# chaitjo/efficient-gnns

Hardware: NVIDIA H100
Metric: edges aggregated/s (fwd+bwd), 3-layer GCN student + logit-KD, ARXIV-shape (higher is better)
Workload: dtype f32

## Files before the change

### efficient-gnns_b200/csrc/common.cuh

```cuda
#pragma once
#include <cuda_runtime.h>
#include <stdint.h>

#include "b200gnn.h"

namespace b200gnn {

void set_cuda_error(cudaError_t e);
void count_launch(int n = 1);

inline int check_launch() {
  cudaError_t e = cudaGetLastError();
  if (e != cudaSuccess) {
    set_cuda_error(e);
    return B200GNN_ERR_CUDA;
  }
  count_launch();
  return B200GNN_OK;
}

constexpr unsigned FULL_MASK = 0xffffffffu;

__device__ __forceinline__ void adam_update(float& p, float& m, float& v, float g, float b1, float b2, float eps,
                                            float step_size, float inv_sqrt_bc2) {
  const float mi = b1 * m + (1.f - b1) * g;
  const float vi = b2 * v + (1.f - b2) * g * g;
  m = mi; v = vi;
  p -= step_size * mi / (sqrtf(vi) * inv_sqrt_bc2 + eps);
}

template <typename V> struct VecTraits;
template <> struct VecTraits<float> { static constexpr int W = 1; };
template <> struct VecTraits<float2> { static constexpr int W = 2; };
template <> struct VecTraits<float4> { static constexpr int W = 4; };

__device__ __forceinline__ void vzero(float& a) { a = 0.f; }
__device__ __forceinline__ void vzero(float2& a) { a.x = a.y = 0.f; }
__device__ __forceinline__ void vzero(float4& a) { a.x = a.y = a.z = a.w = 0.f; }

__device__ __forceinline__ void vfma(float& acc, float s, const float& x) { acc = fmaf(s, x, acc); }
__device__ __forceinline__ void vfma(float2& acc, float s, const float2& x) {
  acc.x = fmaf(s, x.x, acc.x); acc.y = fmaf(s, x.y, acc.y);
}
__device__ __forceinline__ void vfma(float4& acc, float s, const float4& x) {
  acc.x = fmaf(s, x.x, acc.x); acc.y = fmaf(s, x.y, acc.y);
  acc.z = fmaf(s, x.z, acc.z); acc.w = fmaf(s, x.w, acc.w);
}
__device__ __forceinline__ void vadd(float& a, const float& b) { a += b; }
__device__ __forceinline__ void vadd(float2& a, const float2& b) { a.x += b.x; a.y += b.y; }
__device__ __forceinline__ void vadd(float4& a, const float4& b) {
  a.x += b.x; a.y += b.y; a.z += b.z; a.w += b.w;
}
__device__ __forceinline__ void vdiv(float& a, float d) { a /= d; }
__device__ __forceinline__ void vdiv(float2& a, float d) { a.x /= d; a.y /= d; }
__device__ __forceinline__ void vdiv(float4& a, float d) { a.x /= d; a.y /= d; a.z /= d; a.w /= d; }
__device__ __forceinline__ void vstat(float& s, float& q, const float& y) { s += y; q = fmaf(y, y, q); }
__device__ __forceinline__ void vstat(float2& s, float2& q, const float2& y) {
  s.x += y.x; s.y += y.y; q.x = fmaf(y.x, y.x, q.x); q.y = fmaf(y.y, y.y, q.y);
}
__device__ __forceinline__ void vstat(float4& s, float4& q, const float4& y) {
  s.x += y.x; s.y += y.y; s.z += y.z; s.w += y.w;
  q.x = fmaf(y.x, y.x, q.x); q.y = fmaf(y.y, y.y, q.y);
  q.z = fmaf(y.z, y.z, q.z); q.w = fmaf(y.w, y.w, q.w);
}

__device__ __forceinline__ float vshfl_down(float v, int d) { return __shfl_down_sync(FULL_MASK, v, d); }
__device__ __forceinline__ float2 vshfl_down(float2 v, int d) {
  return make_float2(__shfl_down_sync(FULL_MASK, v.x, d), __shfl_down_sync(FULL_MASK, v.y, d));
}
__device__ __forceinline__ float4 vshfl_down(float4 v, int d) {
  return make_float4(__shfl_down_sync(FULL_MASK, v.x, d), __shfl_down_sync(FULL_MASK, v.y, d),
                     __shfl_down_sync(FULL_MASK, v.z, d), __shfl_down_sync(FULL_MASK, v.w, d));
}

__device__ __forceinline__ float vldg(const float* p) { return __ldg(p); }
__device__ __forceinline__ float2 vldg(const float2* p) { return __ldg(p); }
__device__ __forceinline__ float4 vldg(const float4* p) { return __ldg(p); }

__device__ __forceinline__ void vstcs(float* p, const float& v) { __stcs(p, v); }
__device__ __forceinline__ void vstcs(float2* p, const float2& v) { __stcs(p, v); }
__device__ __forceinline__ void vstcs(float4* p, const float4& v) { __stcs(p, v); }

static __global__ void __launch_bounds__(256) sum_partials_kernel(const float* __restrict__ partial, int n, double scale,
                                                                  float* __restrict__ out) {
  __shared__ double s[256];
  double a = 0.0;
  for (int i = threadIdx.x; i < n; i += 256) a += (double)partial[i];
  s[threadIdx.x] = a;
  __syncthreads();
  for (int d = 128; d > 0; d >>= 1) {
    if (threadIdx.x < d) s[threadIdx.x] += s[threadIdx.x + d];
    __syncthreads();
  }
  if (threadIdx.x == 0) out[0] = (float)(s[0] * scale);
}

inline bool aligned_to(const void* p, size_t a) { return (reinterpret_cast<uintptr_t>(p) % a) == 0; }

}
```

### efficient-gnns_b200/csrc/dense_rows.cu

```cuda
#include "common.cuh"
#include "philox.cuh"

namespace b200gnn {

constexpr int ROWS_THREADS = 256;

struct RowMap {
  int nvec, rows_per_iter, cv, rg;
  bool active;
};
__device__ __forceinline__ RowMap make_row_map(int K) {
  RowMap m;
  m.nvec = K >> 2;
  m.rows_per_iter = ROWS_THREADS / m.nvec;
  m.rg = threadIdx.x / m.nvec;
  m.cv = threadIdx.x - m.rg * m.nvec;
  m.active = m.rg < m.rows_per_iter;
  return m;
}

__device__ __forceinline__ float4 ld4(const float* p) { return *reinterpret_cast<const float4*>(p); }
__device__ __forceinline__ float4 ld4s(const float* p) { return __ldcs(reinterpret_cast<const float4*>(p)); }
__device__ __forceinline__ void st4(float* p, const float4& v) { *reinterpret_cast<float4*>(p) = v; }

__device__ __forceinline__ void reduce_store_2xK(const RowMap& m, int K, float4 a, float4 b, float* smem ,
                                                 float* out) {
  for (int i = threadIdx.x; i < 2 * K; i += ROWS_THREADS) smem[i] = 0.f;
  __syncthreads();
  for (int g = 0; g < m.rows_per_iter; ++g) {
    if (m.active && m.rg == g) {
      float* s = smem + 4 * m.cv;
      float* q = smem + K + 4 * m.cv;
      s[0] += a.x; s[1] += a.y; s[2] += a.z; s[3] += a.w;
      q[0] += b.x; q[1] += b.y; q[2] += b.z; q[3] += b.w;
    }
    __syncthreads();
  }
  for (int i = threadIdx.x; i < 2 * K; i += ROWS_THREADS) out[i] = smem[i];
}

__global__ void __launch_bounds__(ROWS_THREADS) col_stats4_kernel(const float* __restrict__ Y, int64_t n_rows, int K,
                                                                  float* __restrict__ partial, int slots) {
  extern __shared__ float smem[];
  const RowMap m = make_row_map(K);
  const int64_t per = (n_rows + slots - 1) / slots;
  const int64_t r0 = (int64_t)blockIdx.x * per, r1 = min(n_rows, r0 + per);
  float4 s = make_float4(0, 0, 0, 0), q = s;
  if (m.active)
    for (int64_t r = r0 + m.rg; r < r1; r += m.rows_per_iter) {
      const float4 y = ld4(Y + (size_t)r * K + 4 * m.cv);
      vstat(s, q, y);
    }
  reduce_store_2xK(m, K, s, q, smem, partial + (size_t)blockIdx.x * 2 * K);
}

constexpr int FIN_COLS = 4, FIN_GROUPS = 64;
__device__ __forceinline__ bool finalize_reduce(const float* __restrict__ partial, int slots, int K, bool second,
                                                double& s_out, double& q_out, int& k_out) {
  __shared__ double sh[2][FIN_GROUPS][FIN_COLS];
  const int c = threadIdx.x % FIN_COLS, g = threadIdx.x / FIN_COLS;
  const int k = blockIdx.x * FIN_COLS + c;
  double s = 0.0, q = 0.0;
  if (k < K)
    for (int j = g; j < slots; j += FIN_GROUPS) {
      s += (double)partial[(size_t)j * 2 * K + k];
      if (second) q += (double)partial[(size_t)j * 2 * K + K + k];
    }
  sh[0][g][c] = s; sh[1][g][c] = q;
  __syncthreads();
  if (g == 0 && k < K) {
    s = 0.0; q = 0.0;
    for (int j = 0; j < FIN_GROUPS; ++j) { s += sh[0][j][c]; q += sh[1][j][c]; }
    s_out = s; q_out = q; k_out = k;
    return true;
  }
  return false;
}

__global__ void __launch_bounds__(256) bn_finalize_kernel(const float* __restrict__ partial, int slots, int K,
                                                          int64_t n, const float* __restrict__ gamma,
                                                          const float* __restrict__ beta, float eps, float momentum,
                                                          float* running_mean, float* running_var, float* mean_out,
                                                          float* invstd_out, float* scale_out, float* shift_out) {
  double s, q; int k;
  if (finalize_reduce(partial, slots, K, true, s, q, k)) {
    const double mean = s / (double)n;
    double var = q / (double)n - mean * mean;
    if (var < 0.0) var = 0.0;
    const float invstd = (float)(1.0 / sqrt(var + (double)eps));
    const float sc = gamma[k] * invstd;
    mean_out[k] = (float)mean;
    invstd_out[k] = invstd;
    scale_out[k] = sc;
    shift_out[k] = beta[k] - (float)mean * sc;
    if (running_mean) {
      const double unbiased = n > 1 ? var * (double)n / (double)(n - 1) : var;
      running_mean[k] = (1.f - momentum) * running_mean[k] + momentum * (float)mean;
      running_var[k] = (1.f - momentum) * running_var[k] + momentum * (float)unbiased;
    }
  }
}

__device__ __forceinline__ float4 affine_relu4(float4 y, const float* __restrict__ scale, const float* __restrict__ shift,
                                               int cv, int relu) {
  if (scale) {
    const float4 sc = ld4(scale + 4 * cv), sh = ld4(shift + 4 * cv);
    y.x = fmaf(y.x, sc.x, sh.x); y.y = fmaf(y.y, sc.y, sh.y);
    y.z = fmaf(y.z, sc.z, sh.z); y.w = fmaf(y.w, sc.w, sh.w);
  }
  if (relu) { y.x = fmaxf(y.x, 0.f); y.y = fmaxf(y.y, 0.f); y.z = fmaxf(y.z, 0.f); y.w = fmaxf(y.w, 0.f); }
  return y;
}

template <bool P16>
__global__ void __launch_bounds__(256) affine_relu_dropout_kernel(const float* __restrict__ Y, float* __restrict__ out,
                                                                  int64_t n_vec, int nvec_row,
                                                                  const float* __restrict__ scale,
                                                                  const float* __restrict__ shift, int relu, float p,
                                                                  uint32_t thr16, uint64_t seed, uint64_t offset,
                                                                  const int32_t* __restrict__ step_dev,
                                                                  uint64_t step_mul, uint64_t index_offset) {
  const float inv_keep = p > 0.f ? 1.f / (1.f - p) : 1.f;
  if (step_dev) offset += (uint64_t)(*step_dev) * step_mul;
  const int64_t tid = (int64_t)blockIdx.x * blockDim.x + threadIdx.x, stride = (int64_t)gridDim.x * blockDim.x;
  if (P16) {
    const uint64_t g0 = index_offset, g1 = index_offset + (uint64_t)n_vec;
    for (uint64_t b = (g0 >> 1) + (uint64_t)tid; b < ((g1 + 1) >> 1); b += (uint64_t)stride) {
      const uint4 r = philox4x32(seed, offset, b);
#pragma unroll
      for (int half = 0; half < 2; ++half) {
        const uint64_t g = 2 * b + half;
        if (g < g0 || g >= g1) continue;
        const int64_t i = (int64_t)(g - g0);
        float4 y = affine_relu4(ld4s(Y + 4 * i), scale, shift, (int)(i % nvec_row), relu);
        const uchar4 m = keep16(half ? r.z : r.x, half ? r.w : r.y, thr16);
        y.x = m.x ? y.x * inv_keep : 0.f; y.y = m.y ? y.y * inv_keep : 0.f;
        y.z = m.z ? y.z * inv_keep : 0.f; y.w = m.w ? y.w * inv_keep : 0.f;
        st4(out + 4 * i, y);
      }
    }
  } else {
    for (int64_t i = tid; i < n_vec; i += stride) {
      float4 y = affine_relu4(ld4s(Y + 4 * i), scale, shift, (int)(i % nvec_row), relu);
      if (p > 0.f) {
        const uchar4 m = keep24(philox4x32(seed, offset, (uint64_t)i + index_offset), p);
        y.x = m.x ? y.x * inv_keep : 0.f; y.y = m.y ? y.y * inv_keep : 0.f;
        y.z = m.z ? y.z * inv_keep : 0.f; y.w = m.w ? y.w * inv_keep : 0.f;
      }
      st4(out + 4 * i, y);
    }
  }
}

struct RowScatter {
  float* ptr[16];
  int32_t off[17];
  int32_t n;
  int64_t ld, col;
};
__device__ __forceinline__ float* scatter_row(const RowScatter& sc, int64_t r) {
  int q = 0;
#pragma unroll 1
  while (q + 1 < sc.n && r >= sc.off[q + 1]) ++q;
  return sc.ptr[q] + (size_t)(r - sc.off[q]) * (size_t)sc.ld + sc.col;
}

template <bool P16>
__global__ void __launch_bounds__(256) affine_relu_dropout_mapped_kernel(
    const float* __restrict__ Y, float* __restrict__ out, int64_t n_rows, int nvec_l, const float* __restrict__ scale,
    const float* __restrict__ shift, int relu, float p, uint32_t thr16, uint64_t seed, uint64_t offset,
    const int32_t* __restrict__ step_dev, uint64_t step_mul, const int32_t* __restrict__ rowmap, uint64_t row_offset,
    uint64_t nvec_g, uint64_t cv_off, int paired, const RowScatter sc) {
  const float inv_keep = p > 0.f ? 1.f / (1.f - p) : 1.f;
  if (step_dev) offset += (uint64_t)(*step_dev) * step_mul;
  const int64_t tid = (int64_t)blockIdx.x * blockDim.x + threadIdx.x, stride = (int64_t)gridDim.x * blockDim.x;
  if (P16 && paired) {
    const int half_l = nvec_l >> 1;
    for (int64_t u = tid; u < n_rows * half_l; u += stride) {
      const int64_t r = u / half_l;
      const int cv = (int)(u - r * half_l) * 2;
      const uint64_t gid = rowmap ? (uint64_t)rowmap[r] : (uint64_t)r + row_offset;
      const uint64_t g = gid * nvec_g + cv_off + (uint64_t)cv;
      const uint4 rnd = philox4x32(seed, offset, g >> 1);
#pragma unroll
      for (int half = 0; half < 2; ++half) {
        const int64_t i = r * nvec_l + cv + half;
        float4 y = affine_relu4(ld4s(Y + 4 * i), scale, shift, cv + half, relu);
        const uchar4 m = keep16(half ? rnd.z : rnd.x, half ? rnd.w : rnd.y, thr16);
        y.x = m.x ? y.x * inv_keep : 0.f; y.y = m.y ? y.y * inv_keep : 0.f;
        y.z = m.z ? y.z * inv_keep : 0.f; y.w = m.w ? y.w * inv_keep : 0.f;
        st4(out + 4 * i, y);
        if (sc.n) st4(scatter_row(sc, r) + 4 * (cv + half), y);
      }
    }
    return;
  }
  for (int64_t i = tid; i < n_rows * nvec_l; i += stride) {
    const int64_t r = i / nvec_l;
    const int cv = (int)(i - r * nvec_l);
    float4 y = affine_relu4(ld4s(Y + 4 * i), scale, shift, cv, relu);
    if (p > 0.f) {
      const uint64_t gid = rowmap ? (uint64_t)rowmap[r] : (uint64_t)r + row_offset;
      const uint64_t g = gid * nvec_g + cv_off + (uint64_t)cv;
      uchar4 m;
      if (P16) {
        const uint4 rnd = philox4x32(seed, offset, g >> 1);
        m = keep16((g & 1) ? rnd.z : rnd.x, (g & 1) ? rnd.w : rnd.y, thr16);
      } else {
        m = keep24(philox4x32(seed, offset, g), p);
      }
      y.x = m.x ? y.x * inv_keep : 0.f; y.y = m.y ? y.y * inv_keep : 0.f;
      y.z = m.z ? y.z * inv_keep : 0.f; y.w = m.w ? y.w * inv_keep : 0.f;
    }
    st4(out + 4 * i, y);
    if (sc.n) st4(scatter_row(sc, r) + 4 * cv, y);
  }
}

__global__ void __launch_bounds__(256) dropout_mask_kernel(uint8_t* __restrict__ mask, int64_t n_vec, float p, int p16,
                                                           uint32_t thr16, uint64_t seed, uint64_t offset) {
  for (int64_t i = (int64_t)blockIdx.x * blockDim.x + threadIdx.x; i < n_vec; i += (int64_t)gridDim.x * blockDim.x) {
    uchar4 m;
    if (p16) {
      const uint4 r = philox4x32(seed, offset, (uint64_t)i >> 1);
      m = keep16((i & 1) ? r.z : r.x, (i & 1) ? r.w : r.y, thr16);
    } else {
      m = keep24(philox4x32(seed, offset, (uint64_t)i), p);
    }
    reinterpret_cast<uchar4*>(mask)[i] = m;
  }
}

__global__ void __launch_bounds__(256) dropout_bits_kernel(uint32_t* __restrict__ bits, int n_layers, int64_t n_rows, int nvec_row,
                                                           int words, float p, int p16, uint32_t thr16, uint64_t seed,
                                                           uint64_t offset, const int32_t* __restrict__ step_dev,
                                                           uint64_t step_mul) {
  if (step_dev) offset += (uint64_t)(*step_dev) * step_mul;
  const int64_t per_layer = n_rows * words;
  for (int64_t t = (int64_t)blockIdx.x * blockDim.x + threadIdx.x; t < per_layer * n_layers; t += (int64_t)gridDim.x * blockDim.x) {
    const int layer = (int)(t / per_layer);
    const int64_t e = t - layer * per_layer, row = e / words;
    const int w = (int)(e - row * words);
    const uint64_t off = offset + (uint64_t)layer;
    uint32_t out = 0u;
    uint64_t blk = ~0ull;
    uint4 r = make_uint4(0u, 0u, 0u, 0u);
#pragma unroll
    for (int j = 0; j < 8; ++j) {
      const int cv = 8 * w + j;
      if (cv >= nvec_row) break;
      const uint64_t g = (uint64_t)row * nvec_row + cv;
      uchar4 m;
      if (p16) {
        if ((g >> 1) != blk) { blk = g >> 1; r = philox4x32(seed, off, blk); }
        m = keep16((g & 1) ? r.z : r.x, (g & 1) ? r.w : r.y, thr16);
      } else {
        m = keep24(philox4x32(seed, off, g), p);
      }
      out |= ((uint32_t)m.x | ((uint32_t)m.y << 1) | ((uint32_t)m.z << 2) | ((uint32_t)m.w << 3)) << (4 * j);
    }
    bits[t] = out;
  }
}

__global__ void __launch_bounds__(256) affine_relu_bits_kernel(const float* __restrict__ Y, const uint32_t* __restrict__ bits,
                                                               const float* __restrict__ scale, const float* __restrict__ shift,
                                                               float* __restrict__ out, int64_t n_vec, int nvec_row, int words,
                                                               float p) {
  const float inv_keep = p > 0.f ? 1.f / (1.f - p) : 1.f;
  for (int64_t i = (int64_t)blockIdx.x * blockDim.x + threadIdx.x; i < n_vec; i += (int64_t)gridDim.x * blockDim.x) {
    const int64_t row = i / nvec_row;
    const int cv = (int)(i - row * nvec_row);
    float4 y = affine_relu4(ld4(Y + 4 * i), scale, shift, cv, 1);
    const uint32_t b = bits[row * words + (cv >> 3)] >> (4 * (cv & 7));
    y.x = (b & 1u) ? y.x * inv_keep : 0.f; y.y = (b & 2u) ? y.y * inv_keep : 0.f;
    y.z = (b & 4u) ? y.z * inv_keep : 0.f; y.w = (b & 8u) ? y.w * inv_keep : 0.f;
    st4(out + 4 * i, y);
  }
}

__global__ void __launch_bounds__(256) relu_dropout_bwd_kernel(const float4* __restrict__ dOut, const float4* __restrict__ Xout,
                                                               float4* dY, int64_t n_vec, float inv_keep) {
  for (int64_t i = (int64_t)blockIdx.x * blockDim.x + threadIdx.x; i < n_vec; i += (int64_t)gridDim.x * blockDim.x) {
    const float4 g = dOut[i], x = Xout[i];
    float4 d;
    d.x = x.x > 0.f ? g.x * inv_keep : 0.f; d.y = x.y > 0.f ? g.y * inv_keep : 0.f;
    d.z = x.z > 0.f ? g.z * inv_keep : 0.f; d.w = x.w > 0.f ? g.w * inv_keep : 0.f;
    dY[i] = d;
  }
}

__global__ void __launch_bounds__(ROWS_THREADS) bn_act_bwd_reduce_kernel(
    const float* __restrict__ dOut, const float* __restrict__ Xout, const float* __restrict__ Y,
    const float* __restrict__ mean, const float* __restrict__ invstd, int64_t n_rows, int K, float inv_keep,
    float* __restrict__ partial, int slots) {
  extern __shared__ float smem[];
  const RowMap m = make_row_map(K);
  const int64_t per = (n_rows + slots - 1) / slots;
  const int64_t r0 = (int64_t)blockIdx.x * per, r1 = min(n_rows, r0 + per);
  float4 s = make_float4(0, 0, 0, 0), q = s;
  if (m.active) {
    const float4 mu = ld4(mean + 4 * m.cv), is = ld4(invstd + 4 * m.cv);
    for (int64_t r = r0 + m.rg; r < r1; r += m.rows_per_iter) {
      const size_t o = (size_t)r * K + 4 * m.cv;
      const float4 g = ld4(dOut + o), x = ld4(Xout + o), y = ld4(Y + o);
      const float dx = x.x > 0.f ? g.x * inv_keep : 0.f, dy = x.y > 0.f ? g.y * inv_keep : 0.f;
      const float dz = x.z > 0.f ? g.z * inv_keep : 0.f, dw = x.w > 0.f ? g.w * inv_keep : 0.f;
      s.x += dx; s.y += dy; s.z += dz; s.w += dw;
      q.x = fmaf(dx, (y.x - mu.x) * is.x, q.x); q.y = fmaf(dy, (y.y - mu.y) * is.y, q.y);
      q.z = fmaf(dz, (y.z - mu.z) * is.z, q.z); q.w = fmaf(dw, (y.w - mu.w) * is.w, q.w);
    }
  }
  reduce_store_2xK(m, K, s, q, smem, partial + (size_t)blockIdx.x * 2 * K);
}

__global__ void __launch_bounds__(256) bn_bwd_finalize_kernel(const float* __restrict__ partial, int slots, int K,
                                                              int64_t n, const float* __restrict__ gamma,
                                                              const float* __restrict__ invstd, float* dgamma,
                                                              float* dbeta, float* coef ) {
  double s, q; int k;
  if (finalize_reduce(partial, slots, K, true, s, q, k)) {
    dbeta[k] = (float)s;
    dgamma[k] = (float)q;
    coef[k] = gamma[k] * invstd[k];
    coef[K + k] = (float)(s / (double)n);
    coef[2 * K + k] = (float)(q / (double)n);
  }
}

template <bool DZ>
__global__ void __launch_bounds__(ROWS_THREADS) bn_act_bwd_apply_kernel(
    const float* __restrict__ dOut, const float* __restrict__ Xout, const float* __restrict__ Y,
    const float* __restrict__ mean, const float* __restrict__ invstd, const float* __restrict__ coef, int64_t n_rows,
    int K, float inv_keep, float* __restrict__ dY, float* __restrict__ colsum_partial, int slots) {
  extern __shared__ float smem[];
  const RowMap m = make_row_map(K);
  const int64_t per = (n_rows + slots - 1) / slots;
  const int64_t r0 = (int64_t)blockIdx.x * per, r1 = min(n_rows, r0 + per);
  float4 s = make_float4(0, 0, 0, 0), q = s;
  if (m.active) {
    const float4 mu = ld4(mean + 4 * m.cv), is = ld4(invstd + 4 * m.cv);
    const float4 c1 = ld4(coef + 4 * m.cv), c2 = ld4(coef + K + 4 * m.cv), c3 = ld4(coef + 2 * K + 4 * m.cv);
    for (int64_t r = r0 + m.rg; r < r1; r += m.rows_per_iter) {
      const size_t o = (size_t)r * K + 4 * m.cv;
      float4 g = ld4s(dOut + o);
      const float4 y = ld4s(Y + o);
      if (!DZ) {
        const float4 x = ld4s(Xout + o);
        g.x = x.x > 0.f ? g.x * inv_keep : 0.f; g.y = x.y > 0.f ? g.y * inv_keep : 0.f;
        g.z = x.z > 0.f ? g.z * inv_keep : 0.f; g.w = x.w > 0.f ? g.w * inv_keep : 0.f;
      }
      float4 d;
      d.x = c1.x * (g.x - c2.x - (y.x - mu.x) * is.x * c3.x);
      d.y = c1.y * (g.y - c2.y - (y.y - mu.y) * is.y * c3.y);
      d.z = c1.z * (g.z - c2.z - (y.z - mu.z) * is.z * c3.z);
      d.w = c1.w * (g.w - c2.w - (y.w - mu.w) * is.w * c3.w);
      st4(dY + o, d);
      s.x += d.x; s.y += d.y; s.z += d.z; s.w += d.w;
    }
  }
  if (colsum_partial) reduce_store_2xK(m, K, s, q, smem, colsum_partial + (size_t)blockIdx.x * 2 * K);
}

__global__ void __launch_bounds__(256) partial_reduce_kernel(const float* __restrict__ partial, int slots, int K2,
                                                             float* __restrict__ out) {
  __shared__ double sh[FIN_GROUPS][FIN_COLS];
  const int c = threadIdx.x % FIN_COLS, g = threadIdx.x / FIN_COLS;
  const int k = blockIdx.x * FIN_COLS + c;
  double s = 0.0;
  if (k < K2)
    for (int j = g; j < slots; j += FIN_GROUPS) s += (double)partial[(size_t)j * K2 + k];
  sh[g][c] = s;
  __syncthreads();
  if (g == 0 && k < K2) {
    s = 0.0;
    for (int j = 0; j < FIN_GROUPS; ++j) s += sh[j][c];
    out[k] = (float)s;
  }
}

__global__ void __launch_bounds__(256) colsum_finalize_kernel(const float* __restrict__ partial, int slots, int K,
                                                              float* __restrict__ out) {
  double s, q; int k;
  if (finalize_reduce(partial, slots, K, false, s, q, k)) out[k] = (float)s;
}

__global__ void __launch_bounds__(256) adam_kernel(float* __restrict__ p, const float* __restrict__ g,
                                                   float* __restrict__ m, float* __restrict__ v, int64_t n, float lr,
                                                   float b1, float b2, float eps, const int32_t* __restrict__ step) {
  const float t = (float)(*step + 1);
  const float bc1 = 1.f - powf(b1, t), bc2 = 1.f - powf(b2, t);
  const float step_size = lr / bc1, inv_sqrt_bc2 = rsqrtf(bc2);
  for (int64_t i = (int64_t)blockIdx.x * blockDim.x + threadIdx.x; i < n; i += (int64_t)gridDim.x * blockDim.x)
    adam_update(p[i], m[i], v[i], g[i], b1, b2, eps, step_size, inv_sqrt_bc2);
}
__global__ void adam_tick_kernel(int32_t* step) { *step += 1; }

static inline int grid_for(int64_t n_items, int per_cta, int cap = 132 * 8) {
  int64_t g = (n_items + per_cta - 1) / per_cta;
  if (g > cap) g = cap;
  if (g < 1) g = 1;
  return (int)g;
}

}

using namespace b200gnn;

static bool rows_ok(int64_t n_rows, int64_t K) { return n_rows >= 0 && K > 0 && K % 4 == 0 && K <= 1024; }

extern "C" int64_t b200gnn_rows_slots(int64_t n_rows) {
  int64_t s = (n_rows + 255) / 256;
  if (s > 132 * 4) s = 132 * 4;
  return s < 1 ? 1 : s;
}

extern "C" int b200gnn_col_stats_f32(const float* Y, int64_t n_rows, int64_t K, float* partial, int64_t slots,
                                     void* stream) {
  if (!rows_ok(n_rows, K) || !Y || !partial || slots < 1 || !aligned_to(Y, 16)) return B200GNN_ERR_BAD_ARG;
  col_stats4_kernel<<<(int)slots, ROWS_THREADS, 2 * K * sizeof(float), (cudaStream_t)stream>>>(Y, n_rows, (int)K, partial,
                                                                                             (int)slots);
  return check_launch();
}

extern "C" int b200gnn_bn_finalize_f32(const float* partial, int64_t slots, int64_t K, int64_t n_rows,
                                       const float* gamma, const float* beta, float eps, float momentum,
                                       float* running_mean, float* running_var, float* mean_out, float* invstd_out,
                                       float* scale_out, float* shift_out, void* stream) {
  if (!partial || slots < 1 || K <= 0 || n_rows <= 0 || !gamma || !beta || !mean_out || !invstd_out || !scale_out ||
      !shift_out || ((running_mean == nullptr) != (running_var == nullptr)))
    return B200GNN_ERR_BAD_ARG;
  bn_finalize_kernel<<<(int)((K + FIN_COLS - 1) / FIN_COLS), 256, 0, (cudaStream_t)stream>>>(
      partial, (int)slots, (int)K, n_rows, gamma, beta, eps, momentum, running_mean, running_var, mean_out, invstd_out,
      scale_out, shift_out);
  return check_launch();
}

extern "C" int b200gnn_affine_relu_dropout_f32(const float* Y, float* out, int64_t n_rows, int64_t K,
                                               const float* scale, const float* shift, int relu, float p, uint64_t seed,
                                               uint64_t offset, const int32_t* step_dev, uint64_t step_mul,
                                               uint64_t row_offset, void* stream) {
  if (!rows_ok(n_rows, K) || !Y || !out || p < 0.f || p >= 1.f || ((scale == nullptr) != (shift == nullptr)) ||
      !aligned_to(Y, 16) || !aligned_to(out, 16))
    return B200GNN_ERR_BAD_ARG;
  if (n_rows == 0) return B200GNN_OK;
  const int64_t n_vec = n_rows * (K / 4);
  uint32_t thr16 = 0;
  if (dropout_p16(p, thr16))
    affine_relu_dropout_kernel<true><<<grid_for((n_vec + 1) / 2 + 1, 256 * 2), 256, 0, (cudaStream_t)stream>>>(
        Y, out, n_vec, (int)(K / 4), scale, shift, relu, p, thr16, seed, offset, step_dev, step_mul,
        row_offset * (uint64_t)(K / 4));
  else
    affine_relu_dropout_kernel<false><<<grid_for(n_vec, 256 * 4), 256, 0, (cudaStream_t)stream>>>(
        Y, out, n_vec, (int)(K / 4), scale, shift, relu, p, 0u, seed, offset, step_dev, step_mul,
        row_offset * (uint64_t)(K / 4));
  return check_launch();
}

static int mapped_launch(const float* Y, float* out, int64_t n_rows, int64_t K, const float* scale, const float* shift, int relu,
                         float p, uint64_t seed, uint64_t offset, const int32_t* step_dev, uint64_t step_mul, const int32_t* rowmap,
                         uint64_t row_offset, int64_t K_global, int64_t col_offset, const RowScatter& sc, void* stream) {
  if (!rows_ok(n_rows, K) || !Y || !out || p < 0.f || p >= 1.f || ((scale == nullptr) != (shift == nullptr)) ||
      !aligned_to(Y, 16) || !aligned_to(out, 16) || K_global < K || K_global % 4 || col_offset < 0 || col_offset % 4 ||
      col_offset + K > K_global)
    return B200GNN_ERR_BAD_ARG;
  if (n_rows == 0) return B200GNN_OK;
  const int nvec_l = (int)(K / 4);
  const uint64_t nvec_g = (uint64_t)(K_global / 4), cv_off = (uint64_t)(col_offset / 4);
  const int paired = (nvec_l % 2 == 0 && nvec_g % 2 == 0 && cv_off % 2 == 0) ? 1 : 0;
  const int64_t n_vec = n_rows * nvec_l;
  uint32_t thr16 = 0;
  if (dropout_p16(p, thr16))
    affine_relu_dropout_mapped_kernel<true><<<grid_for(paired ? n_vec / 2 : n_vec, 256 * 2), 256, 0, (cudaStream_t)stream>>>(
        Y, out, n_rows, nvec_l, scale, shift, relu, p, thr16, seed, offset, step_dev, step_mul, rowmap, row_offset, nvec_g,
        cv_off, paired, sc);
  else
    affine_relu_dropout_mapped_kernel<false><<<grid_for(n_vec, 256 * 4), 256, 0, (cudaStream_t)stream>>>(
        Y, out, n_rows, nvec_l, scale, shift, relu, p, 0u, seed, offset, step_dev, step_mul, rowmap, row_offset, nvec_g,
        cv_off, 0, sc);
  return check_launch();
}

extern "C" int b200gnn_affine_relu_dropout_mapped_f32(const float* Y, float* out, int64_t n_rows, int64_t K,
                                                      const float* scale, const float* shift, int relu, float p,
                                                      uint64_t seed, uint64_t offset, const int32_t* step_dev,
                                                      uint64_t step_mul, const int32_t* rowmap, uint64_t row_offset,
                                                      int64_t K_global, int64_t col_offset, void* stream) {
  RowScatter sc;
  sc.n = 0; sc.ld = 0; sc.col = 0;
  return mapped_launch(Y, out, n_rows, K, scale, shift, relu, p, seed, offset, step_dev, step_mul, rowmap, row_offset, K_global,
                       col_offset, sc, stream);
}

extern "C" int b200gnn_affine_relu_dropout_scatter_f32(const float* Y, float* out, int64_t n_rows, int64_t K,
                                                       const float* scale, const float* shift, int relu, float p,
                                                       uint64_t seed, uint64_t offset, const int32_t* step_dev,
                                                       uint64_t step_mul, const int32_t* rowmap, uint64_t row_offset,
                                                       int64_t K_global, int64_t col_offset, float* const* dst_ptrs,
                                                       const int32_t* row_off, int32_t world, int64_t ld_dst, void* stream) {
  if (!dst_ptrs || !row_off || world <= 0 || world > 16 || ld_dst < K_global || ld_dst % 4 || row_off[0] != 0 ||
      row_off[world] != n_rows)
    return B200GNN_ERR_BAD_ARG;
  RowScatter sc;
  sc.n = world; sc.ld = ld_dst; sc.col = col_offset;
  for (int q = 0; q < world; ++q) {
    if (!dst_ptrs[q] || !aligned_to(dst_ptrs[q], 16) || row_off[q + 1] < row_off[q]) return B200GNN_ERR_BAD_ARG;
    sc.ptr[q] = dst_ptrs[q]; sc.off[q] = row_off[q];
  }
  sc.off[world] = row_off[world];
  return mapped_launch(Y, out, n_rows, K, scale, shift, relu, p, seed, offset, step_dev, step_mul, rowmap, row_offset, K_global,
                       col_offset, sc, stream);
}

extern "C" int b200gnn_dropout_mask_u8(uint8_t* mask, int64_t n_rows, int64_t K, float p, uint64_t seed,
                                       uint64_t offset, void* stream) {
  if (!rows_ok(n_rows, K) || !mask || p < 0.f || p >= 1.f) return B200GNN_ERR_BAD_ARG;
  if (n_rows == 0) return B200GNN_OK;
  const int64_t n_vec = n_rows * (K / 4);
  uint32_t thr16 = 0;
  const int p16 = dropout_p16(p, thr16) ? 1 : 0;
  dropout_mask_kernel<<<grid_for(n_vec, 256 * 4), 256, 0, (cudaStream_t)stream>>>(mask, n_vec, p, p16, thr16, seed, offset);
  return check_launch();
}

extern "C" int b200gnn_dropout_bits_u32(uint32_t* bits, int64_t n_layers, int64_t n_rows, int64_t K, float p, uint64_t seed,
                                        uint64_t offset, const int32_t* step_dev, uint64_t step_mul, void* stream) {
  if (!rows_ok(n_rows, K) || !bits || n_layers < 1 || p < 0.f || p >= 1.f) return B200GNN_ERR_BAD_ARG;
  if (n_rows == 0) return B200GNN_OK;
  const int words = (int)((K + 31) / 32);
  uint32_t thr16 = 0;
  const int p16 = dropout_p16(p, thr16) ? 1 : 0;
  dropout_bits_kernel<<<grid_for(n_layers * n_rows * words, 256 * 2), 256, 0, (cudaStream_t)stream>>>(
      bits, (int)n_layers, n_rows, (int)(K / 4), words, p, p16, thr16, seed, offset, step_dev, step_mul);
  return check_launch();
}

extern "C" int b200gnn_affine_relu_bits_f32(const float* Y, const uint32_t* bits, const float* scale, const float* shift,
                                            float p, float* out, int64_t n_rows, int64_t K, void* stream) {
  if (!rows_ok(n_rows, K) || !Y || !bits || !scale || !shift || !out || p < 0.f || p >= 1.f || !aligned_to(Y, 16) ||
      !aligned_to(out, 16) || !aligned_to(scale, 16) || !aligned_to(shift, 16))
    return B200GNN_ERR_BAD_ARG;
  if (n_rows == 0) return B200GNN_OK;
  const int64_t n_vec = n_rows * (K / 4);
  affine_relu_bits_kernel<<<grid_for(n_vec, 256 * 4), 256, 0, (cudaStream_t)stream>>>(Y, bits, scale, shift, out, n_vec,
                                                                                     (int)(K / 4), (int)((K + 31) / 32), p);
  return check_launch();
}

extern "C" int b200gnn_relu_dropout_bwd_f32(const float* dOut, const float* Xout, float* dY, int64_t n_rows, int64_t K,
                                            float p, void* stream) {
  if (!rows_ok(n_rows, K) || p < 0.f || p >= 1.f) return B200GNN_ERR_BAD_ARG;
  if (n_rows == 0) return B200GNN_OK;
  if (!dOut || !Xout || !dY || !aligned_to(dOut, 16) || !aligned_to(Xout, 16) || !aligned_to(dY, 16)) return B200GNN_ERR_BAD_ARG;
  const int64_t n_vec = n_rows * (K / 4);
  const float inv_keep = p > 0.f ? 1.f / (1.f - p) : 1.f;
  relu_dropout_bwd_kernel<<<grid_for(n_vec, 256 * 4), 256, 0, (cudaStream_t)stream>>>(
      reinterpret_cast<const float4*>(dOut), reinterpret_cast<const float4*>(Xout), reinterpret_cast<float4*>(dY), n_vec, inv_keep);
  return check_launch();
}

extern "C" int b200gnn_bn_act_bwd_reduce_f32(const float* dOut, const float* Xout, const float* Y, const float* mean,
                                             const float* invstd, int64_t n_rows, int64_t K, float p, float* partial,
                                             int64_t slots, void* stream) {
  if (!rows_ok(n_rows, K) || n_rows == 0 || !dOut || !Xout || !Y || !mean || !invstd || !partial || slots < 1 ||
      p < 0.f || p >= 1.f)
    return B200GNN_ERR_BAD_ARG;
  if (ROWS_THREADS / (K / 4) < 1) return B200GNN_ERR_UNSUPPORTED;
  const float inv_keep = p > 0.f ? 1.f / (1.f - p) : 1.f;
  bn_act_bwd_reduce_kernel<<<(int)slots, ROWS_THREADS, 2 * K * sizeof(float), (cudaStream_t)stream>>>(
      dOut, Xout, Y, mean, invstd, n_rows, (int)K, inv_keep, partial, (int)slots);
  return check_launch();
}

extern "C" int b200gnn_bn_act_bwd_apply_f32(const float* dOut, const float* Xout, const float* Y, const float* mean,
                                            const float* invstd, const float* gamma, const float* sums,
                                            int64_t sum_slots, int64_t n_norm, int64_t n_rows, int64_t K, float p,
                                            float* dY, float* dgamma, float* dbeta, float* dbias, float* partial,
                                            int64_t slots, float* coef, void* stream) {
  if (!rows_ok(n_rows, K) || n_rows == 0 || !dOut || !Y || !mean || !invstd || !gamma || !sums || !dY ||
      !dgamma || !dbeta || !partial || !coef || slots < 1 || sum_slots < 1 || n_norm < 1 || p < 0.f || p >= 1.f)
    return B200GNN_ERR_BAD_ARG;
  cudaStream_t st = (cudaStream_t)stream;
  const float inv_keep = p > 0.f ? 1.f / (1.f - p) : 1.f;
  const size_t smem = 2 * K * sizeof(float);
  int rc;
  bn_bwd_finalize_kernel<<<(int)((K + FIN_COLS - 1) / FIN_COLS), 256, 0, st>>>(sums, (int)sum_slots, (int)K, n_norm, gamma,
                                                                              invstd, dgamma, dbeta, coef);
  if ((rc = check_launch())) return rc;
  if (Xout)
    bn_act_bwd_apply_kernel<false><<<(int)slots, ROWS_THREADS, smem, st>>>(dOut, Xout, Y, mean, invstd, coef, n_rows, (int)K,
                                                                          inv_keep, dY, dbias ? partial : nullptr, (int)slots);
  else
    bn_act_bwd_apply_kernel<true><<<(int)slots, ROWS_THREADS, smem, st>>>(dOut, nullptr, Y, mean, invstd, coef, n_rows, (int)K,
                                                                         inv_keep, dY, dbias ? partial : nullptr, (int)slots);
  if ((rc = check_launch())) return rc;
  if (dbias) {
    colsum_finalize_kernel<<<(int)((K + FIN_COLS - 1) / FIN_COLS), 256, 0, st>>>(partial, (int)slots, (int)K, dbias);
    if ((rc = check_launch())) return rc;
  }
  return B200GNN_OK;
}

extern "C" int b200gnn_bn_act_bwd_f32(const float* dOut, const float* Xout, const float* Y, const float* mean,
                                      const float* invstd, const float* gamma, int64_t n_rows, int64_t K, float p,
                                      float* dY, float* dgamma, float* dbeta, float* dbias, float* partial,
                                      int64_t slots, float* coef, void* stream) {
  int rc = b200gnn_bn_act_bwd_reduce_f32(dOut, Xout, Y, mean, invstd, n_rows, K, p, partial, slots, stream);
  if (rc) return rc;
  return b200gnn_bn_act_bwd_apply_f32(dOut, Xout, Y, mean, invstd, gamma, partial, slots, n_rows, n_rows, K, p, dY,
                                      dgamma, dbeta, dbias, partial, slots, coef, stream);
}

extern "C" int b200gnn_partial_reduce_f32(const float* partial, int64_t slots, int64_t K2, float* out, void* stream) {
  if (!partial || !out || slots < 1 || K2 < 1) return B200GNN_ERR_BAD_ARG;
  partial_reduce_kernel<<<(int)((K2 + FIN_COLS - 1) / FIN_COLS), 256, 0, (cudaStream_t)stream>>>(partial, (int)slots, (int)K2,
                                                                                               out);
  return check_launch();
}

extern "C" int b200gnn_col_sum_f32(const float* Y, int64_t n_rows, int64_t K, float* out, float* partial,
                                   int64_t slots, void* stream) {
  if (!rows_ok(n_rows, K) || !Y || !out || !partial || slots < 1) return B200GNN_ERR_BAD_ARG;
  cudaStream_t st = (cudaStream_t)stream;
  int rc;
  col_stats4_kernel<<<(int)slots, ROWS_THREADS, 2 * K * sizeof(float), st>>>(Y, n_rows, (int)K, partial, (int)slots);
  if ((rc = check_launch())) return rc;
  colsum_finalize_kernel<<<(int)((K + FIN_COLS - 1) / FIN_COLS), 256, 0, st>>>(partial, (int)slots, (int)K, out);
  return check_launch();
}

extern "C" int b200gnn_adam_step_f32(float* params, const float* grads, float* exp_avg, float* exp_avg_sq, int64_t n,
                                     float lr, float beta1, float beta2, float eps, int32_t* step, void* stream) {
  if (!params || !grads || !exp_avg || !exp_avg_sq || !step || n < 0) return B200GNN_ERR_BAD_ARG;
  cudaStream_t st = (cudaStream_t)stream;
  int rc;
  if (n > 0) {
    adam_kernel<<<grid_for(n, 256), 256, 0, st>>>(params, grads, exp_avg, exp_avg_sq, n, lr, beta1, beta2, eps, step);
    if ((rc = check_launch())) return rc;
  }
  adam_tick_kernel<<<1, 1, 0, st>>>(step);
  return check_launch();
}
```

### efficient-gnns_b200/csrc/gemm_wgrad_tf32x3.cu

```cuda
#include "common.cuh"
#include "tc_common.cuh"

namespace b200gnn {
namespace wgrad {
using namespace tc;

constexpr int BKN = 32;
constexpr int TM = 128, TN = 128;
constexpr int THREADS = 384;
constexpr int STAGES = 5;
constexpr int X_BOX = 8;
constexpr int RAW_BYTES = BKN * (TM + TN) * 4;
constexpr int OP_BYTES = 128 * BKN * 4;
constexpr int T_BYTES = 2 * OP_BYTES;
constexpr int SS_BYTES = TM / 2 * 16;
constexpr int SMEM_BYTES = STAGES * RAW_BYTES + 2 * T_BYTES + 256 + SS_BYTES + 1024;
constexpr int MAX_RANGES = 132;
constexpr int64_t MAX_PARTIAL_FLOATS = (int64_t)MAX_RANGES * 256 * 256;
constexpr int MAX_KIN = 2048, MAX_NOUT = 512;
static_assert(SMEM_BYTES <= 232448, "shared memory");

struct Params {
  float* partial;
  int32_t Nn, Kin, Kpad, Nout, Npad, num_kb;
  int32_t n_tn, n_ranges;
  const float* act_scale;
  const float* act_shift;
  const uint32_t* act_bits;
  int32_t act_words;
  float inv_keep;
  const float* act_slope;
  int32_t act_ld;
};

template <bool ACT, bool PRELU = false>
__global__ void __launch_bounds__(THREADS, 1)
wgrad_tf32x3_kernel(const __grid_constant__ CUtensorMap tmX, const __grid_constant__ CUtensorMap tmG, const Params p) {
  extern __shared__ uint8_t smem_raw[];
  uint8_t* smem = reinterpret_cast<uint8_t*>((reinterpret_cast<uintptr_t>(smem_raw) + 1023) & ~(uintptr_t)1023);
  uint8_t* tbuf = smem + STAGES * RAW_BYTES;
  uint64_t* full = reinterpret_cast<uint64_t*>(tbuf + 2 * T_BYTES);
  uint64_t* empty = full + STAGES;
  float4* act_ss = reinterpret_cast<float4*>(tbuf + 2 * T_BYTES + 256);

  const int tiles = (p.Kpad / TM) * p.n_tn;
  const int tile = (int)blockIdx.x % tiles, range = (int)blockIdx.x / tiles;
  const int mt = tile / p.n_tn, nt = tile % p.n_tn;
  const int kb0 = (int)((int64_t)p.num_kb * range / p.n_ranges);
  const int kb1 = (int)((int64_t)p.num_kb * (range + 1) / p.n_ranges);

  const int warp = threadIdx.x >> 5, lane = threadIdx.x & 31;
  if (threadIdx.x == 0) {
    for (int s = 0; s < STAGES; ++s) { mbar_init(&full[s], 1); mbar_init(&empty[s], 256); }
    asm volatile("fence.mbarrier_init.release.cluster;" ::: "memory");
  }
  __syncthreads();

  if (warp < 4) {
    regs_dec<40>();
    if (threadIdx.x == 0) {
      int s = 0; uint32_t ph = 0;
      for (int kb = kb0; kb < kb1; ++kb) {
        mbar_wait(&empty[s], ph ^ 1);
        uint8_t* st = smem + s * RAW_BYTES;
        mbar_expect_tx(&full[s], RAW_BYTES);
        for (int j = 0; j < TM / X_BOX; ++j)
          tma_load_2d(&tmX, &full[s], st + j * BKN * X_BOX * 4, mt * TM + j * X_BOX, kb * BKN);
        tma_load_2d(&tmG, &full[s], st + BKN * TM * 4, nt * TN, kb * BKN);
        if (++s == STAGES) { s = 0; ph ^= 1; }
      }
    }
    return;
  }
  regs_inc<232>();

  const int cw = (warp >> 2) - 1;
  const int ct = threadIdx.x - 128;
  const uint32_t xfrag = (8 * cw + 2 * (warp & 3)) * (BKN * X_BOX * 4) + (lane & 3) * (X_BOX * 4) + (lane >> 2) * 4;
  const int pair = cw * 32 + (warp & 3) * 8 + (lane >> 2);
  const int c0 = mt * TM + cw * 64 + (warp & 3) * 16 + (lane >> 2);
  uint32_t wnext = 0u;
  const int bits_ld = PRELU ? p.act_ld : p.act_words;
  auto act_word = [&](int kb) {
    const int node = kb * BKN + lane;
    return node < p.Nn && (c0 >> 5) < p.act_words ? __ldg(p.act_bits + (size_t)node * bits_ld + (c0 >> 5)) : 0u;
  };
  const float slope = PRELU ? __ldg(p.act_slope) : 0.f;
  if (PRELU && kb0 < kb1) wnext = act_word(kb0);
  if (ACT) {
    if (ct < TM / 2) {
      const int c = mt * TM + (ct >> 3) * 16 + (ct & 7);
      float4 v = make_float4(0.f, 0.f, 0.f, 0.f);
      if (c < p.Kin) { v.x = __ldg(p.act_scale + c); v.y = __ldg(p.act_shift + c); }
      if (c + 8 < p.Kin) { v.z = __ldg(p.act_scale + c + 8); v.w = __ldg(p.act_shift + c + 8); }
      act_ss[ct] = v;
    }
    if (kb0 < kb1) wnext = act_word(kb0);
    named_sync(1, 256);
  }
  float acc[64], sum[64];
#pragma unroll
  for (int i = 0; i < 64; ++i) sum[i] = acc[i] = 0.f;
  uint32_t xh0[BKN / 8][4], xl0[BKN / 8][4], xh1[BKN / 8][4], xl1[BKN / 8][4];
  int s = 0; uint32_t ph = 0;
  auto block = [&](int i, uint32_t (&h)[BKN / 8][4], uint32_t (&l)[BKN / 8][4]) {
    uint32_t wcur = 0u;
    if (ACT || PRELU) {
      wcur = wnext;
      if (kb0 + i + 1 < kb1) wnext = act_word(kb0 + i + 1);
    }
    mbar_wait(&full[s], ph);
    float4 ss = make_float4(0.f, 0.f, 0.f, 0.f);
    int l4 = lane & 3;
    if (ACT) {
      ss = act_ss[pair];
      asm volatile("" : "+r"(l4));
    }
    if (PRELU) asm volatile("" : "+r"(l4));
    const uint32_t sraw = smem_u32(smem + s * RAW_BYTES);
    const float* rg = reinterpret_cast<const float*>(smem + s * RAW_BYTES + BKN * TM * 4);
    uint8_t* T = tbuf + (i & 1) * T_BYTES;
#pragma unroll
    for (int u = 0; u < 4; ++u) {
      const int idx = u * 256 + ct;
      const int r = idx & 127, c = idx >> 7;
      const float* src = rg + (4 * c) * 128 + r;
      const uint4 v = make_uint4(__float_as_uint(src[0]), __float_as_uint(src[128]), __float_as_uint(src[256]),
                                 __float_as_uint(src[384]));
      uint4 hv, lv;
      split4(v, hv, lv);
      *reinterpret_cast<uint4*>(T + swz128(r, c)) = hv;
      *reinterpret_cast<uint4*>(T + OP_BYTES + swz128(r, c)) = lv;
    }
#pragma unroll
    for (int k = 0; k < BKN / 8; ++k)
#pragma unroll
      for (int j = 0; j < 4; ++j) {
        uint32_t v = lds32(sraw + xfrag + (j & 1) * (BKN * X_BOX * 4) + (8 * k + 4 * (j >> 1)) * (X_BOX * 4));
        if (ACT) {
          const uint32_t w = __shfl_sync(0xffffffffu, wcur, 8 * k + l4 + 4 * (j >> 1));
          const float y = fmaxf(fmaf(__uint_as_float(v), (j & 1) ? ss.z : ss.x, (j & 1) ? ss.w : ss.y), 0.f) * p.inv_keep;
          v = (w >> ((c0 & 31) + 8 * (j & 1))) & 1u ? __float_as_uint(y) : 0u;
        }
        if (PRELU) {
          const uint32_t w = __shfl_sync(0xffffffffu, wcur, 8 * k + l4 + 4 * (j >> 1));
          const float z = __uint_as_float(v);
          const float y = (z > 0.f ? z : slope * z) * p.inv_keep;
          v = (w >> ((c0 & 31) + 8 * (j & 1))) & 1u ? __float_as_uint(y) : 0u;
        }
        split1(v, h[k][j], l[k][j]);
      }
    asm volatile("fence.proxy.async.shared::cta;" ::: "memory");
    mbar_arrive(&empty[s]);
    if (i > 0) {
      wgmma_wait<0>();
      acc_fence(acc);
#pragma unroll
      for (int j = 0; j < 64; ++j) sum[j] += acc[j];
    }
    named_sync(1, 256);
    reg_fence(h); reg_fence(l);
    wgmma_fence();
    const uint32_t sa = smem_u32(T);
#pragma unroll
    for (int k = 0; k < BKN / 8; ++k) {
      const uint32_t koff = k * 32;
      wgmma_tf32_n128_rs(acc, l[k], make_desc_k128(sa + koff), k != 0);
      wgmma_tf32_n128_rs(acc, h[k], make_desc_k128(sa + OP_BYTES + koff), 1);
    }
#pragma unroll
    for (int k = 0; k < BKN / 8; ++k) wgmma_tf32_n128_rs(acc, h[k], make_desc_k128(sa + k * 32), 1);
    wgmma_commit();
    if (++s == STAGES) { s = 0; ph ^= 1; }
  };
  for (int i = 0; i < kb1 - kb0; i += 2) {
    block(i, xh0, xl0);
    if (i + 1 < kb1 - kb0) block(i + 1, xh1, xl1);
  }
  if (kb1 > kb0) {
    wgmma_wait<0>();
    acc_fence(acc);
#pragma unroll
    for (int j = 0; j < 64; ++j) sum[j] += acc[j];
  }
  float* out = p.partial + (size_t)range * p.Kpad * p.Npad;
  const int row0 = mt * TM + cw * 64 + (warp & 3) * 16 + (lane >> 2);
#pragma unroll
  for (int j = 0; j < 16; ++j) {
    const int col = nt * TN + 8 * j + 2 * (lane & 3);
    if (col < p.Npad) {
      *reinterpret_cast<float2*>(out + (size_t)row0 * p.Npad + col) = make_float2(sum[4 * j], sum[4 * j + 1]);
      *reinterpret_cast<float2*>(out + (size_t)(row0 + 8) * p.Npad + col) = make_float2(sum[4 * j + 2], sum[4 * j + 3]);
    }
  }
}

constexpr int RED_VECS = 32, RED_GROUPS = 8;
__global__ void __launch_bounds__(RED_VECS * RED_GROUPS) wgrad_reduce_kernel(const float4* __restrict__ partial, int n_part,
                                                                             int Kin, int Kpad, int Nout, int Npad,
                                                                             float* __restrict__ out) {
  __shared__ float4 sh[RED_GROUPS][RED_VECS];
  const int64_t n_vec = (int64_t)Kpad * Npad / 4;
  const int v = threadIdx.x % RED_VECS, g = threadIdx.x / RED_VECS;
  const int64_t i = (int64_t)blockIdx.x * RED_VECS + v;
  float4 acc = make_float4(0.f, 0.f, 0.f, 0.f);
  if (i < n_vec)
    for (int c = g; c < n_part; c += RED_GROUPS) {
      const float4 x = __ldcs(partial + (size_t)c * n_vec + i);
      acc.x += x.x; acc.y += x.y; acc.z += x.z; acc.w += x.w;
    }
  sh[g][v] = acc;
  __syncthreads();
  if (g != 0 || i >= n_vec) return;
  const int row = (int)(i / (Npad / 4)), c4 = (int)(i % (Npad / 4)) * 4;
  if (c4 >= Nout || row >= Kin) return;
#pragma unroll
  for (int j = 1; j < RED_GROUPS; ++j) {
    const float4 x = sh[j][v];
    acc.x += x.x; acc.y += x.y; acc.z += x.z; acc.w += x.w;
  }
  *reinterpret_cast<float4*>(out + (size_t)row * Nout + c4) = acc;
}

static bool make_map_rows(CUtensorMap* m, const float* base, int64_t rows, int64_t width, int64_t ld, int box_cols) {
  EncodeTiledFn fn = encode_fn();
  if (!fn) return false;
  cuuint64_t dims[2] = {(cuuint64_t)width, (cuuint64_t)rows};
  cuuint64_t strides[1] = {(cuuint64_t)ld * 4};
  cuuint32_t box[2] = {(cuuint32_t)box_cols, (cuuint32_t)BKN};
  cuuint32_t estr[2] = {1, 1};
  return fn(m, CU_TENSOR_MAP_DATA_TYPE_FLOAT32, 2, const_cast<float*>(base), dims, strides, box, estr,
            CU_TENSOR_MAP_INTERLEAVE_NONE, CU_TENSOR_MAP_SWIZZLE_NONE, CU_TENSOR_MAP_L2_PROMOTION_L2_256B,
            CU_TENSOR_MAP_FLOAT_OOB_FILL_NONE) == CUDA_SUCCESS;
}

static int64_t pad_k(int64_t Kin) { return (Kin + TM - 1) / TM * TM; }
static int64_t pad_n(int64_t Nout) { return (Nout + 31) / 32 * 32; }
static int range_cap(int64_t Kin, int64_t Nout) {
  const int64_t c = MAX_PARTIAL_FLOATS / (pad_k(Kin) * pad_n(Nout));
  return (int)(c > MAX_RANGES ? MAX_RANGES : (c < 1 ? 1 : c));
}

}
}

using namespace b200gnn;

extern "C" int64_t b200gnn_wgrad_workspace_floats(int64_t Kin, int64_t Nout) {
  if (Kin <= 0 || Nout <= 0) return B200GNN_ERR_BAD_ARG;
  if (Kin > wgrad::MAX_KIN || Nout > wgrad::MAX_NOUT) return B200GNN_ERR_UNSUPPORTED;
  return wgrad::range_cap(Kin, Nout) * wgrad::pad_k(Kin) * wgrad::pad_n(Nout);
}

template <bool ACT, bool PRELU = false>
static int wgrad_launch(const float* X, int64_t ldx, const float* G, int64_t ldg, float* dW, int64_t Nn, int64_t Kin, int64_t Nout,
                        float* workspace, const wgrad::Params& act, void* stream) {
  if (!X || !G || !dW || !workspace || Nn <= 0 || Kin <= 0 || Nout <= 0 || ldx < Kin || ldg < Nout || Nn >= INT32_MAX)
    return B200GNN_ERR_BAD_ARG;
  if (Kin % 4 || Kin > wgrad::MAX_KIN || Nout % 4 || Nout > wgrad::MAX_NOUT || ldx % 4 || ldg % 4 || !aligned_to(X, 16) || !aligned_to(G, 16) ||
      !aligned_to(dW, 16) || !aligned_to(workspace, 16))
    return B200GNN_ERR_UNSUPPORTED;
  CUtensorMap tX, tG;
  if (!wgrad::make_map_rows(&tX, X, Nn, Kin, ldx, wgrad::X_BOX) || !wgrad::make_map_rows(&tG, G, Nn, Nout, ldg, wgrad::TN))
    return B200GNN_ERR_UNSUPPORTED;
  int dev = 0, sms = 132;
  cudaGetDevice(&dev);
  static bool attr_set[64] = {};
  if (dev >= 0 && dev < 64 && !attr_set[dev]) {
    cudaError_t e = cudaFuncSetAttribute(wgrad::wgrad_tf32x3_kernel<ACT, PRELU>, cudaFuncAttributeMaxDynamicSharedMemorySize,
                                         wgrad::SMEM_BYTES);
    if (e != cudaSuccess) { set_cuda_error(e); return B200GNN_ERR_CUDA; }
    attr_set[dev] = true;
  }
  cudaDeviceGetAttribute(&sms, cudaDevAttrMultiProcessorCount, dev);
  cudaStream_t st = (cudaStream_t)stream;
  wgrad::Params p = act;
  p.partial = workspace; p.Nn = (int32_t)Nn; p.Kin = (int32_t)Kin; p.Nout = (int32_t)Nout;
  p.Kpad = (int32_t)wgrad::pad_k(Kin);
  p.Npad = (int32_t)wgrad::pad_n(Nout);
  p.num_kb = (int32_t)((Nn + wgrad::BKN - 1) / wgrad::BKN);
  p.n_tn = (p.Npad + wgrad::TN - 1) / wgrad::TN;
  const int tiles = (int)(p.Kpad / wgrad::TM) * p.n_tn;
  int ranges = sms / tiles;
  const int cap = wgrad::range_cap(Kin, Nout);
  if (ranges > cap) ranges = cap;
  if (ranges > p.num_kb) ranges = p.num_kb;
  if (ranges < 1) ranges = 1;
  p.n_ranges = ranges;
  int rc;
  wgrad::wgrad_tf32x3_kernel<ACT, PRELU><<<tiles * ranges, wgrad::THREADS, wgrad::SMEM_BYTES, st>>>(tX, tG, p);
  if ((rc = check_launch())) return rc;
  const int64_t n_vec = (int64_t)p.Kpad * p.Npad / 4;
  wgrad::wgrad_reduce_kernel<<<(int)((n_vec + wgrad::RED_VECS - 1) / wgrad::RED_VECS), wgrad::RED_VECS * wgrad::RED_GROUPS, 0, st>>>(
      reinterpret_cast<const float4*>(workspace), ranges, (int)Kin, p.Kpad, (int)Nout, p.Npad, dW);
  return check_launch();
}

extern "C" int b200gnn_gemm_wgrad_tf32x3_f32(const float* X, int64_t ldx, const float* G, int64_t ldg, float* dW,
                                             int64_t Nn, int64_t Kin, int64_t Nout, float* workspace, void* stream) {
  return wgrad_launch<false>(X, ldx, G, ldg, dW, Nn, Kin, Nout, workspace, wgrad::Params{}, stream);
}

extern "C" int b200gnn_gemm_wgrad_tf32x3_act_f32(const float* Y, int64_t ldx, const float* G, int64_t ldg, float* dW,
                                                 int64_t Nn, int64_t Kin, int64_t Nout, const float* scale, const float* shift,
                                                 const uint32_t* bits, float p_drop, float* workspace, void* stream) {
  if (!scale || !shift || !bits || p_drop < 0.f || p_drop >= 1.f) return B200GNN_ERR_BAD_ARG;
  wgrad::Params act{};
  act.act_scale = scale; act.act_shift = shift; act.act_bits = bits; act.act_words = (int32_t)((Kin + 31) / 32);
  act.inv_keep = p_drop > 0.f ? 1.f / (1.f - p_drop) : 1.f;
  return wgrad_launch<true>(Y, ldx, G, ldg, dW, Nn, Kin, Nout, workspace, act, stream);
}

extern "C" int b200gnn_gemm_wgrad_tf32x3_prelu_f32(const float* Z, int64_t ldz, const float* G, int64_t ldg, float* dW,
                                                   int64_t Nn, int64_t Kin, int64_t Nout, const float* slope,
                                                   const uint32_t* bits, int64_t ldbits, float p_drop, float* workspace,
                                                   void* stream) {
  if (!slope || !bits || ldbits < (Kin + 31) / 32 || ldbits >= INT32_MAX || p_drop < 0.f || p_drop >= 1.f)
    return B200GNN_ERR_BAD_ARG;
  wgrad::Params act{};
  act.act_slope = slope; act.act_bits = bits; act.act_words = (int32_t)((Kin + 31) / 32); act.act_ld = (int32_t)ldbits;
  act.inv_keep = p_drop > 0.f ? 1.f / (1.f - p_drop) : 1.f;
  return wgrad_launch<false, true>(Z, ldz, G, ldg, dW, Nn, Kin, Nout, workspace, act, stream);
}
```

### efficient-gnns_b200/engine.py

```python
from __future__ import annotations

import math
from typing import Dict, List, Optional

import torch

from . import lib, ops
from .sparse import CsrGraph, SparseTensor


def gcn_norm(adj: SparseTensor) -> SparseTensor:
    if not adj.has_value():
        adj = adj.fill_value(1.0)
    adj = adj.fill_diag(1.0)
    deg = adj.sum(dim=1)
    dis = deg.pow(-0.5)
    dis.masked_fill_(dis == float("inf"), 0.0)
    row, col, val = adj.coo()
    return adj.set_value(dis[row] * val * dis[col])


def _is_symmetric(adj: SparseTensor) -> bool:
    st = adj.storage
    if st.sparse_sizes()[0] != st.sparse_sizes()[1]:
        return False
    perm = st.csr2csc()
    same = torch.equal(st.col()[perm], st.row()) and torch.equal(st.row()[perm], st.col())
    if same and st.value() is not None:
        same = torch.equal(st.value()[perm], st.value())
    return bool(same)


class GCNStudentTrainer:

    def __init__(self, adj: SparseTensor, dims: List[int], dropout: float = 0.5, lr: float = 0.01, seed: int = 0,
                 alpha: float = 0.9, kd_T: float = 4.0, bn_eps: float = 1e-5, bn_momentum: float = 0.1,
                 aggregate_first: Optional[bool] = None, tensor_core_gemm: bool = True, overlap_wgrad: bool = True,
                 fuse_row_passes: bool = True, fuse_activations: bool = True, _prebuilt_graph: Optional[CsrGraph] = None, _rows_alloc: Optional[int] = None):
        assert adj.is_cuda(), "the engine runs on a CUDA device"
        self.device = adj.device
        self.dims, self.L = list(dims), len(dims) - 1
        self.p, self.lr, self.alpha, self.kd_T = float(dropout), float(lr), float(alpha), float(kd_T)
        self.bn_eps, self.bn_momentum = bn_eps, bn_momentum
        self.seed = int(seed)
        self.tc_gemm = bool(tensor_core_gemm) and all(d % 4 == 0 for d in dims)
        for d in dims[1:]:
            assert d % 4 == 0 and d <= 1024, "layer widths must be multiples of 4 (128-bit rows)"
        self.N = adj.size(0)
        self.agg_first = (dims[0] < dims[1] and dims[0] % 4 == 0) if aggregate_first is None else bool(aggregate_first)
        if self.L < 2:
            self.agg_first = False

        if _prebuilt_graph is not None:
            self.G = self.Gt = _prebuilt_graph
            self.N = _prebuilt_graph.n_rows
        else:
            norm = gcn_norm(adj)
            self.G: CsrGraph = norm.storage.engine_csr()
            self.Gt: CsrGraph = self.G if _is_symmetric(norm) else norm.storage.engine_csc("value")
        self.nnz = self.G.nnz

        sizes = []
        for l in range(self.L):
            sizes += [dims[l] * dims[l + 1], dims[l + 1]]
            if l < self.L - 1:
                sizes += [dims[l + 1], dims[l + 1]]
        n_par = sum(sizes)
        dev = self.device
        self.params = torch.zeros(n_par, device=dev)
        self.n_par_pad = (n_par + 3) // 4 * 4
        self._grads_buf = torch.zeros(self.n_par_pad + 4, device=dev)
        self.grads = self._grads_buf[:n_par]
        self.exp_avg = torch.zeros(n_par, device=dev)
        self.exp_avg_sq = torch.zeros(n_par, device=dev)
        self.step_count = torch.zeros(1, dtype=torch.int32, device=dev)
        self.W, self.b, self.gamma, self.beta = [], [], [], []
        self.gW, self.gb, self.ggamma, self.gbeta = [], [], [], []
        off = 0

        def take(n, shape):
            nonlocal off
            v = (self.params[off:off + n].view(shape), self.grads[off:off + n].view(shape))
            off += n
            return v
        for l in range(self.L):
            w, gw = take(dims[l] * dims[l + 1], (dims[l], dims[l + 1]))
            b, gb = take(dims[l + 1], (dims[l + 1],))
            self.W.append(w); self.gW.append(gw); self.b.append(b); self.gb.append(gb)
            if l < self.L - 1:
                g, gg = take(dims[l + 1], (dims[l + 1],))
                be, gbe = take(dims[l + 1], (dims[l + 1],))
                self.gamma.append(g); self.ggamma.append(gg); self.beta.append(be); self.gbeta.append(gbe)
        self.Wt_split = [(torch.empty(dims[l + 1], dims[l], device=dev), torch.empty(dims[l + 1], dims[l], device=dev))
                         for l in range(self.L)]
        self.W_split = [(torch.empty(dims[l], dims[l + 1], device=dev), torch.empty(dims[l], dims[l + 1], device=dev))
                        for l in range(self.L)]
        wg = [ops.wgrad_supported(dims[l], dims[l + 1]) for l in range(self.L)]
        self.wgrad_ws = (torch.empty(max(ops.wgrad_workspace_floats(dims[l], dims[l + 1]) for l in range(self.L) if wg[l]), device=dev)
                         if self.tc_gemm and any(wg) else None)
        self.running_mean = [torch.zeros(d, device=dev) for d in dims[1:-1]]
        self.running_var = [torch.ones(d, device=dev) for d in dims[1:-1]]
        self.reset_parameters(seed)

        N = self.N
        rows_alloc = N if _rows_alloc is None else _rows_alloc
        self._blocks = []

        def buf(k):
            blk = torch.zeros(rows_alloc, k, device=dev)
            self._blocks.append(blk)
            return blk[:N]
        self.H = [buf(dims[l + 1]) for l in range(self.L)]
        self.Y = [buf(dims[l + 1]) for l in range(self.L)]
        self._A = [buf(dims[l + 1]) for l in range(self.L - 1)]
        self.dY = [buf(dims[l + 1]) for l in range(self.L)]
        self.dH = [buf(dims[l + 1]) for l in range(self.L)]
        self.dA = [buf(dims[l + 1]) for l in range(self.L - 1)]
        self.AX = buf(dims[0]) if self.agg_first else None
        slots_spmm = ops.stat_slots(self.G)
        self.stat_part = [torch.empty(slots_spmm, 2, dims[l + 1], device=dev) for l in range(self.L - 1)]
        self.bn = [torch.empty(4, dims[l + 1], device=dev) for l in range(self.L - 1)]
        self.rs = ops.rows_slots(N)
        self.fuse_rows = bool(fuse_row_passes) and self.tc_gemm
        self._gemm_part = {k: torch.empty(ops.gemm_stat_slots(N, k), 2, k, device=dev)
                           for k in set(dims[1:-1]) if self.fuse_rows and ops.gemm_stats_supported(k)}
        hid = dims[1:-1]
        self.fuse_act = (bool(fuse_activations) and self.fuse_rows and self.L >= 2 and len(set(hid)) == 1
                         and ops.gemm_stats_supported(hid[0]) and hid[0] <= 2048
                         and all(ops.wgrad_supported(dims[l], dims[l + 1]) for l in range(1, self.L)))
        self.keep_bits = (torch.zeros(self.L - 1, N, (hid[0] + 31) // 32, dtype=torch.int32, device=dev)
                          if self.fuse_act else None)
        self._act_stale = False
        self._fwd_fused = False
        self._ev_bits = torch.cuda.Event()
        self.loss_out = self._grads_buf[self.n_par_pad:self.n_par_pad + 3]
        self.kd_part = torch.empty(2 * int(lib.load().b200gnn_kd_partials(N)), device=dev)
        self._graph = None
        self.overlap_wgrad = overlap_wgrad
        self._side = torch.cuda.Stream(device=dev) if overlap_wgrad else None
        self._ev_fork, self._ev_join = torch.cuda.Event(), torch.cuda.Event()
        self._static: Dict[str, torch.Tensor] = {}
        for k in set(dims[1:]):
            self._part(k); self._coef(k)

    def reset_parameters(self, seed: int = 0):
        g = torch.Generator().manual_seed(seed)
        for l in range(self.L):
            fan_in, fan_out = self.dims[l], self.dims[l + 1]
            a = math.sqrt(6.0 / (fan_in + fan_out))
            self.W[l].copy_((torch.rand(fan_in, fan_out, generator=g) * 2 - 1) * a)
            self.b[l].zero_()
        for l in range(self.L - 1):
            self.gamma[l].fill_(1.0); self.beta[l].zero_()
            self.running_mean[l].zero_(); self.running_var[l].fill_(1.0)
        self.exp_avg.zero_(); self.exp_avg_sq.zero_(); self.step_count.zero_()

    def state_dict(self) -> Dict[str, torch.Tensor]:
        sd = {}
        for l in range(self.L):
            sd[f"convs.{l}.weight"] = self.W[l].detach().clone()
            sd[f"convs.{l}.bias"] = self.b[l].detach().clone()
        for l in range(self.L - 1):
            sd[f"bns.{l}.weight"] = self.gamma[l].detach().clone()
            sd[f"bns.{l}.bias"] = self.beta[l].detach().clone()
            sd[f"bns.{l}.running_mean"] = self.running_mean[l].clone()
            sd[f"bns.{l}.running_var"] = self.running_var[l].clone()
        return sd

    def load_state_dict(self, sd: Dict[str, torch.Tensor]):
        for l in range(self.L):
            self.W[l].copy_(sd[f"convs.{l}.weight"]); self.b[l].copy_(sd[f"convs.{l}.bias"])
        for l in range(self.L - 1):
            self.gamma[l].copy_(sd[f"bns.{l}.weight"]); self.beta[l].copy_(sd[f"bns.{l}.bias"])
            if f"bns.{l}.running_mean" in sd:
                self.running_mean[l].copy_(sd[f"bns.{l}.running_mean"]); self.running_var[l].copy_(sd[f"bns.{l}.running_var"])

    @property
    def A(self) -> List[torch.Tensor]:
        if self._act_stale:
            self._act_stale = False
            for l in range(self.L - 1):
                ops.affine_relu_bits(self.Y[l], self.keep_bits[l], self.bn[l][2], self.bn[l][3], self.p, out=self._A[l])
        return self._A

    def _act(self, l: int):
        return self.Y[l], self.bn[l][2], self.bn[l][3], self.keep_bits[l]

    def activation_pattern(self, l: int) -> torch.Tensor:
        return self.A[l] > 0

    def out_feat(self) -> torch.Tensor:
        return self.A[-1]

    def dropout_offset(self, layer: int, step: int) -> int:
        return layer + step * self.L

    def forward(self, x: torch.Tensor, training: bool = True) -> torch.Tensor:
        fused = training and self.fuse_act
        self._act_stale = False
        if fused:
            if self._side is not None:
                self._ev_fork.record(torch.cuda.current_stream())
                self._side.wait_event(self._ev_fork)
                with torch.cuda.stream(self._side):
                    ops.dropout_bits(self.keep_bits, self.p, self.seed, 0, step_dev=self.step_count, step_mul=self.L)
                self._ev_bits.record(self._side)
            else:
                ops.dropout_bits(self.keep_bits, self.p, self.seed, 0, step_dev=self.step_count, step_mul=self.L)
        A = self._A
        inp = x
        for l in range(self.L):
            last = l == self.L - 1
            if l == 0 and self.agg_first:
                ops.spmm_csr(self.G, x, "sum", out=self.AX)
                if training:
                    gp = self._gemm_part.get(self.dims[1])
                    if gp is not None:
                        hi, lo = ops.split_tf32(self.W[0], transpose=True, hi=self.Wt_split[0][0], lo=self.Wt_split[0][1])
                        ops.gemm_tf32x3_stats(self.AX, hi, lo, self.b[0], self.Y[0], gp)
                        part = gp
                    else:
                        self._linear(0, self.AX, self.Y[0], bias=self.b[0])
                        part = ops.col_stats(self.Y[0], partial=self._part(self.dims[1]))
                    ops.bn_finalize(part, self.N, self.gamma[0], self.beta[0], self.bn_eps,
                                    self.bn_momentum, self.running_mean[0], self.running_var[0], out=self.bn[0])
                    if not fused:
                        ops.affine_relu_dropout(self.Y[0], self.bn[0][2], self.bn[0][3], True, self.p, self.seed, 0,
                                                out=A[0], step_dev=self.step_count, step_mul=self.L)
                else:
                    self._linear(0, self.AX, self.Y[0], bias=self.b[0])
                    scale = self.gamma[0] * torch.rsqrt(self.running_var[0] + self.bn_eps)
                    shift = self.beta[0] - self.running_mean[0] * scale
                    ops.affine_relu_dropout(self.Y[0], scale, shift, True, 0.0, out=A[0])
                inp = A[0]
                continue
            if fused and l > 0:
                if l == 1 and self._side is not None:
                    torch.cuda.current_stream().wait_event(self._ev_bits)
                self._linear(l, None, self.H[l], act=self._act(l - 1))
            else:
                self._linear(l, inp, self.H[l])
            if last:
                ops.spmm_csr(self.G, self.H[l], "sum", bias=self.b[l], out=self.Y[l])
            elif training:
                ops.spmm_csr(self.G, self.H[l], "sum", bias=self.b[l], out=self.Y[l], stat_partial=self.stat_part[l])
                ops.bn_finalize(self.stat_part[l], self.N, self.gamma[l], self.beta[l], self.bn_eps, self.bn_momentum,
                                self.running_mean[l], self.running_var[l], out=self.bn[l])
                if not fused:
                    ops.affine_relu_dropout(self.Y[l], self.bn[l][2], self.bn[l][3], True, self.p, self.seed, l,
                                            out=A[l], step_dev=self.step_count, step_mul=self.L)
                inp = A[l]
            else:
                ops.spmm_csr(self.G, self.H[l], "sum", bias=self.b[l], out=self.Y[l])
                scale = self.gamma[l] * torch.rsqrt(self.running_var[l] + self.bn_eps)
                shift = self.beta[l] - self.running_mean[l] * scale
                ops.affine_relu_dropout(self.Y[l], scale, shift, True, 0.0, out=A[l])
                inp = A[l]
        self._act_stale = self._fwd_fused = fused
        return self.Y[-1]

    def backward(self, x: torch.Tensor, d_out_feat: Optional[torch.Tensor] = None):
        fused = self._fwd_fused
        for l in range(self.L - 1, -1, -1):
            act = self._act(l - 1) if fused and l > 0 else None
            inp = x if l == 0 else (None if act else self._A[l - 1])
            if l == self.L - 1:
                ops.col_sum(self.dY[l], out=self.gb[l], partial=self._part(self.dims[l + 1]))
            if l == 0 and self.agg_first:
                self._wgrad_async(0, self.AX, self.dY[0])
                continue
            ops.spmm_csr(self.Gt, self.dY[l], "sum", out=self.dH[l])
            d_prev = self.dA[l - 1] if l > 0 else None
            gp = self._gemm_part.get(self.dims[l]) if l > 0 else None
            if l > 0:
                acc = d_out_feat is not None and l == self.L - 1
                if acc:
                    d_prev = d_out_feat
                if gp is not None:
                    hi, lo = ops.split_tf32(self.W[l], transpose=False, hi=self.W_split[l][0], lo=self.W_split[l][1])
                    if act:
                        ops.gemm_tf32x3_bnbwd_bits(self.dH[l], hi, lo, d_prev, act[3], self.Y[l - 1], self.bn[l - 1][0],
                                                   self.bn[l - 1][1], act[1], act[2], self.p, gp, accumulate=acc)
                    else:
                        ops.gemm_tf32x3_bnbwd(self.dH[l], hi, lo, d_prev, self._A[l - 1], self.Y[l - 1], self.bn[l - 1][0],
                                              self.bn[l - 1][1], self.p, gp, accumulate=acc)
                else:
                    self._linear_dgrad(l, self.dH[l], d_prev, accumulate=acc)
            self._wgrad_async(l, inp, self.dH[l], act=act)
            if l > 0:
                k = self.dims[l]
                part = self._part(k)
                if gp is not None:
                    ops.bn_act_bwd_apply(d_prev, None, self.Y[l - 1], self.bn[l - 1][0], self.bn[l - 1][1], self.gamma[l - 1],
                                         gp, self.N, self.p, self.dY[l - 1], self.ggamma[l - 1], self.gbeta[l - 1],
                                         self.gb[l - 1], part, self._coef(k))
                else:
                    ops.bn_act_bwd(d_prev, self._A[l - 1], self.Y[l - 1], self.bn[l - 1][0], self.bn[l - 1][1],
                                   self.gamma[l - 1], self.p, d_y=self.dY[l - 1], d_gamma=self.ggamma[l - 1],
                                   d_beta=self.gbeta[l - 1], d_bias=self.gb[l - 1], partial=part, coef=self._coef(k))
        self._wgrad_join()

    def _wgrad_async(self, l: int, inp: Optional[torch.Tensor], d_out: torch.Tensor, act=None):
        if self._side is None:
            return self._linear_wgrad(l, inp, d_out, act)
        self._ev_fork.record(torch.cuda.current_stream())
        self._side.wait_event(self._ev_fork)
        with torch.cuda.stream(self._side):
            self._linear_wgrad(l, inp, d_out, act)

    def _wgrad_join(self):
        if self._side is not None:
            self._ev_join.record(self._side)
            torch.cuda.current_stream().wait_event(self._ev_join)

    def _linear(self, l: int, inp: Optional[torch.Tensor], out: torch.Tensor, bias: Optional[torch.Tensor] = None, act=None):
        if act is not None:
            hi, lo = ops.split_tf32(self.W[l], transpose=True, hi=self.Wt_split[l][0], lo=self.Wt_split[l][1])
            ops.gemm_tf32x3_act(*act, self.p, hi, lo, bias=bias, out=out)
        elif self.tc_gemm:
            hi, lo = ops.split_tf32(self.W[l], transpose=True, hi=self.Wt_split[l][0], lo=self.Wt_split[l][1])
            ops.gemm_tf32x3(inp, hi, lo, bias=bias, out=out)
        elif bias is not None:
            torch.addmm(bias, inp, self.W[l], out=out)
        else:
            torch.mm(inp, self.W[l], out=out)

    def _linear_dgrad(self, l: int, d_out: torch.Tensor, d_inp: torch.Tensor, accumulate: bool = False):
        if self.tc_gemm:
            hi, lo = ops.split_tf32(self.W[l], transpose=False, hi=self.W_split[l][0], lo=self.W_split[l][1])
            ops.gemm_tf32x3(d_out, hi, lo, out=d_inp, accumulate=accumulate)
        elif accumulate:
            d_inp.addmm_(d_out, self.W[l].t())
        else:
            torch.mm(d_out, self.W[l].t(), out=d_inp)

    def _linear_wgrad(self, l: int, inp: Optional[torch.Tensor], d_out: torch.Tensor, act=None):
        if act is not None:
            ops.gemm_wgrad_tf32x3_act(*act, self.p, d_out, out=self.gW[l], workspace=self.wgrad_ws)
        elif self.tc_gemm and ops.wgrad_supported(self.dims[l], self.dims[l + 1]):
            ops.gemm_wgrad_tf32x3(inp, d_out, out=self.gW[l], workspace=self.wgrad_ws)
        else:
            torch.mm(inp.t(), d_out, out=self.gW[l])

    def _part(self, k: int) -> torch.Tensor:
        key = f"part{k}"
        if key not in self._static:
            self._static[key] = torch.empty(self.rs, 2, k, device=self.device)
        return self._static[key]

    def _coef(self, k: int) -> torch.Tensor:
        key = f"coef{k}"
        if key not in self._static:
            self._static[key] = torch.empty(3, k, device=self.device)
        return self._static[key]

    def _step_impl(self, x, y, train_idx, teacher_logits):
        logits = self.forward(x, training=True)
        self.dY[-1].zero_()
        ops.kd_loss_fwd_bwd(logits, y, train_idx, teacher_logits, self.alpha, self.kd_T, d_logits=self.dY[-1],
                            loss_out=self.loss_out, partial=self.kd_part)
        self.backward(x)
        ops.adam_step(self.params, self.grads, self.exp_avg, self.exp_avg_sq, self.step_count, self.lr)

    def train_step(self, x, y, train_idx, teacher_logits=None, aux=None, beta: float = 1.0) -> torch.Tensor:
        if aux is None:
            self._step_impl(x, y, train_idx, teacher_logits)
            return self.loss_out
        logits = self.forward(x, training=True)
        self.dY[-1].zero_()
        ops.kd_loss_fwd_bwd(logits, y, train_idx, teacher_logits, self.alpha, self.kd_T, d_logits=self.dY[-1],
                            loss_out=self.loss_out, partial=self.kd_part)
        feat = self.out_feat().detach().requires_grad_(True)
        with torch.enable_grad():
            loss_aux = aux(feat)
            (loss_aux * beta).backward()
        d_feat = feat.grad if feat.grad is not None else torch.zeros_like(feat)
        self.backward(x, d_out_feat=d_feat.contiguous())
        ops.adam_step(self.params, self.grads, self.exp_avg, self.exp_avg_sq, self.step_count, self.lr)
        self.loss_aux = loss_aux.detach()
        self.loss_out[0].add_(self.loss_aux * beta)
        return self.loss_out

    def capture(self, x, y, train_idx, teacher_logits=None, warmup: int = 2, key: int = 0):
        self._static.update(x=x, y=y, train_idx=train_idx, teacher=teacher_logits)
        s = torch.cuda.Stream()
        s.wait_stream(torch.cuda.current_stream())
        with torch.cuda.stream(s):
            for _ in range(warmup):
                self._step_impl(x, y, train_idx, teacher_logits)
        torch.cuda.current_stream().wait_stream(s)
        torch.cuda.synchronize()
        if self._graph is None:
            self._graph = {}
        g = torch.cuda.CUDAGraph()
        with torch.cuda.graph(g):
            self._step_impl(x, y, train_idx, teacher_logits)
        self._graph[key] = g
        return self

    def replay(self, key: int = 0) -> torch.Tensor:
        self._graph[key].replay()
        self._act_stale = self.fuse_act
        return self.loss_out

    def launches_per_step(self) -> int:
        before = lib.launch_count()
        st = self._static
        self._step_impl(st["x"], st["y"], st["train_idx"], st["teacher"])
        return lib.launch_count() - before

    def aggregations_per_step(self) -> Dict[int, int]:
        out: Dict[int, int] = {}
        for l in range(self.L):
            if l == 0 and self.agg_first:
                out[self.dims[0]] = out.get(self.dims[0], 0) + 1
            else:
                out[self.dims[l + 1]] = out.get(self.dims[l + 1], 0) + 2
        return out

    def spmm_algorithmic_bytes(self) -> Dict[int, int]:
        return {k: 2 * self.N * k * 4 + self.nnz * 8 + (self.N + 1) * 4 for k in set(self.dims)}
```

### efficient-gnns_b200/lib.py

```python
from __future__ import annotations

import ctypes as C
import os
from pathlib import Path

import torch

PKG_DIR = Path(__file__).resolve().parent
LIB_PATH = PKG_DIR / "libb200gnn.so"

OK = 0
REDUCE_SUM = 0
REDUCE_MEAN = 1

_i32p = C.c_void_p
_f32p = C.c_void_p
_ptr = C.c_void_p
_i64 = C.c_int64
_i32 = C.c_int32
_int = C.c_int
_f32 = C.c_float
_u64 = C.c_uint64

SIGNATURES = {
    "b200gnn_abi_version": (_int, []),
    "b200gnn_error_string": (C.c_char_p, [_int]),
    "b200gnn_last_cuda_error": (C.c_char_p, []),
    "b200gnn_launch_count": (_i64, []),
    "b200gnn_reset_launch_count": (None, []),
    "b200gnn_csr_chunk_count": (_i64, [_i64, _i64, _i32, _i32]),
    "b200gnn_csr_chunk_plan": (_int, [_i32p, _i64, _i64, _i32, _i32, _i32p, _ptr]),
    "b200gnn_csr_hub_count": (_int, [_i32p, _i64, _i32, _i32, _i32p, _ptr]),
    "b200gnn_csr_hub_fill": (_int, [_i32p, _i64, _i32, _i32, _i32p, _i32p, _i64, _ptr]),
    "b200gnn_spmm_stat_slots": (_i64, [_i64, _i64]),
    "b200gnn_spmm_set_variant": (None, [_int]),
    "b200gnn_spmm_csr_f32": (_int, [_i32p, _i32p, _f32p, _f32p, _i64, _f32p, _i64, _i64, _i64, _i64, _int,
                                    _f32p, _f32p, _i32p, _i64, _i32, _i32, _i32p, _i32p, _i64, _i64, _f32p, _ptr]),
    "b200gnn_spmm_csr_scatter_f32": (_int, [_i32p, _i32p, _f32p, _f32p, _i64, _ptr, _ptr, _i32, _i64, _i64, _i64, _i64, _i64, _int,
                                            _f32p, _i32p, _i64, _i32, _i32, _i32p, _i32p, _i64, _i64, _f32p, _ptr]),
    "b200gnn_rows_slots": (_i64, [_i64]),
    "b200gnn_col_stats_f32": (_int, [_f32p, _i64, _i64, _f32p, _i64, _ptr]),
    "b200gnn_col_sum_f32": (_int, [_f32p, _i64, _i64, _f32p, _f32p, _i64, _ptr]),
    "b200gnn_bn_finalize_f32": (_int, [_f32p, _i64, _i64, _i64, _f32p, _f32p, _f32, _f32, _f32p, _f32p,
                                       _f32p, _f32p, _f32p, _f32p, _ptr]),
    "b200gnn_affine_relu_dropout_f32": (_int, [_f32p, _f32p, _i64, _i64, _f32p, _f32p, _int, _f32, _u64, _u64,
                                               _i32p, _u64, _u64, _ptr]),
    "b200gnn_affine_relu_dropout_mapped_f32": (_int, [_f32p, _f32p, _i64, _i64, _f32p, _f32p, _int, _f32, _u64, _u64,
                                                      _i32p, _u64, _i32p, _u64, _i64, _i64, _ptr]),
    "b200gnn_affine_relu_dropout_scatter_f32": (_int, [_f32p, _f32p, _i64, _i64, _f32p, _f32p, _int, _f32, _u64, _u64,
                                                       _i32p, _u64, _i32p, _u64, _i64, _i64, _ptr, _ptr, _i32, _i64, _ptr]),
    "b200gnn_dropout_mask_u8": (_int, [_ptr, _i64, _i64, _f32, _u64, _u64, _ptr]),
    "b200gnn_dropout_bits_u32": (_int, [_ptr, _i64, _i64, _i64, _f32, _u64, _u64, _i32p, _u64, _ptr]),
    "b200gnn_affine_relu_bits_f32": (_int, [_f32p, _ptr, _f32p, _f32p, _f32, _f32p, _i64, _i64, _ptr]),
    "b200gnn_relu_dropout_bwd_f32": (_int, [_f32p, _f32p, _f32p, _i64, _i64, _f32, _ptr]),
    "b200gnn_bn_act_bwd_f32": (_int, [_f32p, _f32p, _f32p, _f32p, _f32p, _f32p, _i64, _i64, _f32, _f32p, _f32p,
                                      _f32p, _f32p, _f32p, _i64, _f32p, _ptr]),
    "b200gnn_bn_act_bwd_reduce_f32": (_int, [_f32p, _f32p, _f32p, _f32p, _f32p, _i64, _i64, _f32, _f32p, _i64, _ptr]),
    "b200gnn_bn_act_bwd_apply_f32": (_int, [_f32p, _f32p, _f32p, _f32p, _f32p, _f32p, _f32p, _i64, _i64, _i64, _i64, _f32,
                                            _f32p, _f32p, _f32p, _f32p, _f32p, _i64, _f32p, _ptr]),
    "b200gnn_partial_reduce_f32": (_int, [_f32p, _i64, _i64, _f32p, _ptr]),
    "b200gnn_adam_step_f32": (_int, [_f32p, _f32p, _f32p, _f32p, _i64, _f32, _f32, _f32, _f32, _i32p, _ptr]),
    "b200gnn_kd_partials": (_i64, [_i64]),
    "b200gnn_kd_loss_fwd_bwd_f32": (_int, [_f32p, _i64, _ptr, _i64, _ptr, _f32p, _i64, _i64, _f32, _f32, _i64, _f32p,
                                           _i64, _f32p, _f32p, _ptr]),
    "b200gnn_split_tf32_f32": (_int, [_f32p, _i64, _i64, _int, _f32p, _f32p, _ptr]),
    "b200gnn_gemm_tf32x3_f32": (_int, [_f32p, _i64, _f32p, _f32p, _i64, _f32p, _i64, _i64, _i64, _i64, _f32p, _ptr]),
    "b200gnn_random_walk_i64": (_int, [_i32p, _i32p, _i64, _ptr, _i64, _i32, _u64, _u64, _ptr, _ptr]),
    "b200gnn_saint_subgraph_count_i64": (_int, [_i32p, _i32p, _ptr, _i64, _i32p, _ptr, _ptr]),
    "b200gnn_saint_subgraph_fill_i64": (_int, [_i32p, _i32p, _ptr, _ptr, _i64, _i32p, _ptr, _ptr, _ptr, _ptr, _ptr]),
    "b200gnn_gemm_stat_slots": (_i64, [_i64, _i64]),
    "b200gnn_gemm_set_bnbwd_variant": (None, [_int]),
    "b200gnn_gemm_tf32x3_stats_f32": (_int, [_f32p, _i64, _f32p, _f32p, _i64, _f32p, _i64, _i64, _i64, _i64, _f32p, _int, _f32p, _i64,
                                             _ptr]),
    "b200gnn_gemm_tf32x3_bnbwd_f32": (_int, [_f32p, _i64, _f32p, _f32p, _i64, _f32p, _i64, _i64, _i64, _i64, _int,
                                             _f32p, _f32p, _f32p, _f32p, _f32, _f32p, _i64, _ptr]),
    "b200gnn_gemm_tf32x3_bnbwd_bits_f32": (_int, [_f32p, _i64, _f32p, _f32p, _i64, _f32p, _i64, _i64, _i64, _i64, _int,
                                                  _ptr, _f32p, _f32p, _f32p, _f32p, _f32p, _f32, _f32p, _i64, _ptr]),
    "b200gnn_gemm_tf32x3_act_f32": (_int, [_f32p, _i64, _f32p, _f32p, _i64, _f32p, _i64, _i64, _i64, _i64, _f32p,
                                           _f32p, _f32p, _ptr, _f32, _ptr]),
    "b200gnn_gemm_tf32x3_acc_f32": (_int, [_f32p, _i64, _f32p, _f32p, _i64, _f32p, _i64, _i64, _i64, _i64, _ptr]),
    "b200gnn_gemm_tf32x3_scatter_f32": (_int, [_f32p, _i64, _f32p, _f32p, _i64, _ptr, _i32, _i64, _i64, _i64, _i64, _f32p, _ptr]),
    "b200gnn_gemm_tf32x3_bcast_f32": (_int, [_f32p, _i64, _f32p, _f32p, _i64, _ptr, _i32, _i64, _i64, _i64, _i64, _i64, _f32p, _ptr]),
    "b200gnn_wgrad_workspace_floats": (_i64, [_i64, _i64]),
    "b200gnn_gemm_wgrad_tf32x3_f32": (_int, [_f32p, _i64, _f32p, _i64, _f32p, _i64, _i64, _i64, _f32p, _ptr]),
    "b200gnn_gemm_wgrad_tf32x3_act_f32": (_int, [_f32p, _i64, _f32p, _i64, _f32p, _i64, _i64, _i64, _f32p, _f32p, _ptr, _f32,
                                                 _f32p, _ptr]),
    "b200gnn_gemm_tf32x3_prelu_f32": (_int, [_f32p, _i64, _f32p, _f32p, _i64, _f32p, _i64, _i64, _i64, _i64, _f32p,
                                             _f32p, _ptr, _f32, _ptr]),
    "b200gnn_gemm_tf32x3_prelu_bwd_f32": (_int, [_f32p, _i64, _f32p, _f32p, _i64, _f32p, _i64, _i64, _i64, _i64, _int,
                                                 _f32p, _ptr, _f32p, _f32, _f32p, _int, _ptr, _i64, _ptr]),
    "b200gnn_gemm_wgrad_tf32x3_prelu_f32": (_int, [_f32p, _i64, _f32p, _i64, _f32p, _i64, _i64, _i64, _f32p, _ptr, _i64, _f32,
                                                   _f32p, _ptr]),
    "b200gnn_prelu_bits_f32": (_int, [_f32p, _i64, _ptr, _i64, _f32p, _f32, _f32p, _i64, _i64, _i64, _ptr]),
    "b200gnn_sign_gather_f32": (_int, [_ptr, _i32, _i64, _i64, _ptr, _i64, _f32, _u64, _u64, _i32p, _u64, _f32p, _ptr, _ptr,
                                       _f32p, _i64, _i64, _f32p, _ptr]),
    "b200gnn_col_sum_ld_slots": (_i64, [_i64]),
    "b200gnn_col_sum_ld_f32": (_int, [_f32p, _i64, _i64, _i64, _f32p, _f32p, _i64, _ptr]),
    "b200gnn_row_normalize_fwd_f32": (_int, [_f32p, _i64, _i64, _f32, _f32, _f32p, _f32p, _ptr]),
    "b200gnn_row_normalize_bwd_f32": (_int, [_f32p, _f32p, _f32p, _i64, _i64, _f32, _f32, _f32p, _int, _ptr]),
    "b200gnn_reduce_slots": (_i64, [_i64]),
    "b200gnn_mse_fwd_bwd_f32": (_int, [_f32p, _f32p, _i64, _f32, _f32p, _f32p, _f32p, _ptr]),
    "b200gnn_bce_logits_fwd_bwd_f32": (_int, [_f32p, _f32p, _int, _i64, _f32, _f32p, _f32p, _f32p, _ptr]),
    "b200gnn_row_sqnorm_f32": (_int, [_f32p, _i64, _i64, _f32p, _ptr]),
    "b200gnn_row_sqnorm_bwd_f32": (_int, [_f32p, _f32p, _i64, _i64, _f32p, _ptr]),
    "b200gnn_nce_rows_f32": (_int, [_f32p, _i64, _f32p, _f32p, _ptr]),
    "b200gnn_nce_rows_chunk_f32": (_int, [_f32p, _i64, _i64, _i64, _i64, _f32p, _ptr]),
    "b200gnn_nce_finish_f32": (_int, [_f32p, _i64, _f32p, _ptr]),
    "b200gnn_transpose_f32": (_int, [_f32p, _i64, _i64, _f32p, _ptr]),
    "b200gnn_gsp_pair_f32": (_int, [_f32p, _f32p, _f32p, _f32p, _i64, _int, _f32p, _f32p, _f32p, _ptr]),
    "b200gnn_row_axpy_f32": (_int, [_f32p, _f32p, _i64, _i64, _f32, _f32p, _ptr]),
    "b200gnn_edge_sim_f32": (_int, [_f32p, _i64, _i32p, _i32p, _i64, _int, _f32p, _ptr]),
    "b200gnn_lsp_partials": (_i64, [_i64]),
    "b200gnn_lsp_segment_f32": (_int, [_f32p, _f32p, _i32p, _i64, _i64, _int, _f32p, _f32p, _f32p, _ptr]),
    "b200gnn_edge_sim_bwd_f32": (_int, [_f32p, _i64, _i32p, _i32p, _i64, _int, _f32p, _f32p, _f32p, _ptr]),
    "b200gnn_lsp_bwd_values_f32": (_int, [_f32p, _i64, _i32p, _i32p, _i64, _int, _f32p, _f32p, _i32p, _i32p, _i32p, _i32p, _i64,
                                          _f32p, _f32p, _ptr]),
    "b200gnn_gat_edge_softmax_f32": (_int, [_i32p, _i32p, _f32p, _f32p, _i64, _i64, _f32, _f32, _f32p, _ptr, _ptr]),
    "b200gnn_gat_aggregate_f32": (_int, [_i32p, _i32p, _i32p, _f32p, _f32p, _i64, _f32p, _i64, _i64, _i64, _i64, _i32p, _i64,
                                         _i32, _i32, _i32p, _i32p, _i64, _i64, _f32p, _ptr]),
    "b200gnn_gat_bwd_rows_f32": (_int, [_i32p, _i32p, _f32p, _f32p, _i64, _f32p, _i64, _f32p, _f32p, _i64, _i64, _i64, _f32,
                                        _f32p, _f32p, _i32p, _i64, _i32, _i32, _i32p, _i32p, _i64, _i64, _f32p, _f32p, _ptr]),
    "b200gnn_segment_sum_heads_f32": (_int, [_i32p, _i32p, _f32p, _i64, _i64, _f32p, _ptr]),
    "b200gnn_graph_sort_workspace_bytes": (_i64, [_i64]),
    "b200gnn_graph_argsort_i64": (_int, [_ptr, _ptr, _i64, _i64, _i64, _i32p, _ptr, _ptr]),
    "b200gnn_graph_coalesce_i64": (_int, [_ptr, _ptr, _i64, _i64, _i64, _ptr, _ptr, _i32p, _ptr, _ptr, _ptr, _ptr]),
    "b200gnn_typed_gather_f32": (_int, [_ptr, _ptr, _i32, _ptr, _ptr, _i64, _i64, _f32p, _i64, _i32p, _ptr]),
    "b200gnn_typed_scatter_f32": (_int, [_f32p, _i64, _ptr, _ptr, _ptr, _i64, _i64, _ptr, _ptr, _i32, _ptr]),
    "b200gnn_embedding_adam_f32": (_int, [_f32p, _i64, _ptr, _ptr, _ptr, _i64, _i64, _f32p, _f32p, _f32p, _i64, _i64, _i32p,
                                          _f32, _f32, _f32, _f32, _i32p, _ptr]),
    "b200gnn_arena_alloc": (_int, [_i64, C.POINTER(C.c_void_p)]),
    "b200gnn_arena_free": (_int, [_ptr]),
    "b200gnn_ipc_get_handle": (_int, [_ptr, _ptr]),
    "b200gnn_ipc_open_handle": (_int, [_ptr, C.POINTER(C.c_void_p)]),
    "b200gnn_ipc_close_handle": (_int, [_ptr]),
    "b200gnn_peer_copy2d_f32": (_int, [_ptr, _i32, _i64, _ptr]),
    "b200gnn_peer_barrier": (_int, [_ptr, _i32, _i32, _ptr, _ptr, _ptr]),
    "b200gnn_peer_exchange_f32": (_int, [_ptr, _i32, _i64, _ptr, _i32, _i32, _ptr, _ptr, _ptr, _ptr]),
}


class Copy2D(C.Structure):
    _fields_ = [("dst", C.c_void_p), ("src", C.c_void_p), ("ld_dst", C.c_int64), ("ld_src", C.c_int64), ("rows", C.c_int64)]

_lib = None


class B200GnnError(RuntimeError):
    pass


def load() -> C.CDLL:
    global _lib
    if _lib is not None:
        return _lib
    if not LIB_PATH.exists():
        raise B200GnnError(
            f"{LIB_PATH} is missing: build it with `python -c 'import __graft_entry__ as g; g.build()'` "
            "(nvcc, sm_90a). There is no CPU or PyTorch fallback for the b200gnn operators.")
    lib = C.CDLL(str(LIB_PATH))
    for name, (res, args) in SIGNATURES.items():
        fn = getattr(lib, name)
        fn.restype = res
        fn.argtypes = args
    if lib.b200gnn_abi_version() != 2:
        raise B200GnnError("libb200gnn.so ABI version mismatch; rebuild")
    _lib = lib
    report = os.environ.get("B200GNN_LAUNCH_REPORT")
    if report:
        import atexit
        atexit.register(lambda: Path(report).write_text(str(int(lib.b200gnn_launch_count()))))
    return lib


def check(rc: int, what: str) -> None:
    if rc != OK:
        lib = load()
        msg = lib.b200gnn_error_string(rc).decode()
        if rc == -3:
            msg += ": " + lib.b200gnn_last_cuda_error().decode()
        raise B200GnnError(f"{what} failed: {msg}")


def stream_ptr() -> int:
    return torch.cuda.current_stream().cuda_stream


def dptr(t: torch.Tensor | None, dtype: torch.dtype, name: str) -> int | None:
    if t is None:
        return None
    if not isinstance(t, torch.Tensor):
        raise TypeError(f"{name}: expected a tensor")
    if not t.is_cuda:
        raise B200GnnError(f"{name}: b200gnn operators need CUDA tensors (got {t.device}); there is no CPU fallback")
    if t.dtype != dtype:
        raise B200GnnError(f"{name}: expected dtype {dtype}, got {t.dtype}")
    if not t.is_contiguous():
        raise B200GnnError(f"{name}: tensor must be contiguous")
    return t.data_ptr()


def launch_count() -> int:
    return int(load().b200gnn_launch_count())


def reset_launch_count() -> None:
    load().b200gnn_reset_launch_count()
```

### efficient-gnns_b200/ops.py

```python
from __future__ import annotations

from typing import Optional, Tuple

import torch

from . import lib
from .sparse import CsrGraph, SparseTensor

_REDUCE = {"sum": lib.REDUCE_SUM, "add": lib.REDUCE_SUM, "mean": lib.REDUCE_MEAN}


def set_spmm_variant(variant: int) -> None:
    lib.load().b200gnn_spmm_set_variant(int(variant))


def stat_slots(g: CsrGraph) -> int:
    return int(lib.load().b200gnn_spmm_stat_slots(g.n_chunks, g.n_hub))


def spmm_csr(g: CsrGraph, x: torch.Tensor, reduce: str = "sum", bias: Optional[torch.Tensor] = None,
             out: Optional[torch.Tensor] = None, stat_partial: Optional[torch.Tensor] = None) -> torch.Tensor:
    if reduce not in _REDUCE:
        raise ValueError(f"reduce={reduce!r}: the engine implements sum/add/mean (what the reference path uses)")
    if x.dim() != 2:
        raise lib.B200GnnError("spmm: dense operand must be [n_src, K]")
    if x.shape[0] < g.n_cols:
        raise lib.B200GnnError(
            f"spmm: dense operand has {x.shape[0]} rows, matrix has {g.n_cols} columns")
    K = x.shape[1]
    if out is None:
        out = torch.empty(g.n_rows, K, dtype=torch.float32, device=x.device)
    if g.n_rows == 0 or K == 0:
        return out
    L = lib.load()
    ws = g.hub_workspace(K)
    rc = L.b200gnn_spmm_csr_f32(
        lib.dptr(g.rowptr, torch.int32, "rowptr"), lib.dptr(g.col, torch.int32, "col"),
        lib.dptr(g.val, torch.float32, "val"), lib.dptr(x, torch.float32, "x"), x.stride(0),
        lib.dptr(out, torch.float32, "out"), out.stride(0), g.n_rows, g.n_cols, K, _REDUCE[reduce],
        lib.dptr(bias, torch.float32, "bias"), lib.dptr(stat_partial, torch.float32, "stat_partial"),
        g.chunk_rowptr.data_ptr(), g.n_chunks, g.hub_threshold, g.seg_len,
        g.hub_rows.data_ptr() if g.n_hub else None, g.hub_segptr.data_ptr() if g.n_hub else None,
        g.n_hub, g.n_seg, None if ws is None else ws.data_ptr(), lib.stream_ptr())
    lib.check(rc, "spmm_csr_f32")
    return out


def _host_ptr_array(ptrs):
    import ctypes as C
    return (C.c_void_p * len(ptrs))(*[C.c_void_p(int(p)) for p in ptrs])


def _host_i32_array(vals):
    import ctypes as C
    return (C.c_int32 * len(vals))(*[int(v) for v in vals])


def spmm_csr_scatter(g: CsrGraph, x: torch.Tensor, dst_ptrs, row_off, ld_dst: int, col_dst: int, reduce: str = "sum",
                     bias: Optional[torch.Tensor] = None) -> None:
    K = x.shape[1]
    L = lib.load()
    ws = g.hub_workspace(K)
    rc = L.b200gnn_spmm_csr_scatter_f32(
        lib.dptr(g.rowptr, torch.int32, "rowptr"), lib.dptr(g.col, torch.int32, "col"), lib.dptr(g.val, torch.float32, "val"),
        lib.dptr(x, torch.float32, "x"), x.stride(0), _host_ptr_array(dst_ptrs), _host_i32_array(row_off), len(dst_ptrs),
        int(ld_dst), int(col_dst), g.n_rows, g.n_cols, K, _REDUCE[reduce], lib.dptr(bias, torch.float32, "bias"),
        g.chunk_rowptr.data_ptr(), g.n_chunks, g.hub_threshold, g.seg_len,
        g.hub_rows.data_ptr() if g.n_hub else None, g.hub_segptr.data_ptr() if g.n_hub else None,
        g.n_hub, g.n_seg, None if ws is None else ws.data_ptr(), lib.stream_ptr())
    lib.check(rc, "spmm_csr_scatter_f32")


class _SpMM(torch.autograd.Function):

    @staticmethod
    def forward(ctx, x, adj: SparseTensor, reduce: str):
        st = adj.storage
        g = st.engine_csr() if st.value() is not None else st.engine_csr_unweighted()
        ctx.adj, ctx.reduce = adj, reduce
        return spmm_csr(g, x.contiguous(), reduce)

    @staticmethod
    def backward(ctx, grad_out):
        st = ctx.adj.storage
        if ctx.reduce == "mean":
            gt = st.engine_csc("mean" if st.value() is None else "mean_value")
        else:
            gt = st.engine_csc("value")
        return spmm_csr(gt, grad_out.contiguous(), "sum"), None, None


def matmul(adj: SparseTensor, x: torch.Tensor, reduce: str = "sum") -> torch.Tensor:
    if reduce not in _REDUCE:
        raise ValueError(f"reduce={reduce!r} not implemented (reference path uses add/mean)")
    v = adj.storage.value()
    if v is not None and v.requires_grad:
        raise NotImplementedError("gradients w.r.t. sparse values are never taken on the reference path")
    if x.dim() == 1:
        return matmul(adj, x.unsqueeze(-1), reduce).squeeze(-1)
    return _SpMM.apply(x, adj, reduce)


def _f32(t, name):
    return lib.dptr(t, torch.float32, name)


def rows_slots(n_rows: int) -> int:
    return int(lib.load().b200gnn_rows_slots(n_rows))


def col_stats(y: torch.Tensor, partial: Optional[torch.Tensor] = None) -> torch.Tensor:
    n, K = y.shape
    slots = rows_slots(n)
    if partial is None:
        partial = torch.empty(slots, 2, K, dtype=torch.float32, device=y.device)
    lib.check(lib.load().b200gnn_col_stats_f32(_f32(y, "y"), n, K, _f32(partial, "partial"), slots, lib.stream_ptr()),
              "col_stats_f32")
    return partial


def col_sum(y: torch.Tensor, out: Optional[torch.Tensor] = None, partial: Optional[torch.Tensor] = None) -> torch.Tensor:
    n, K = y.shape
    slots = rows_slots(n)
    if out is None:
        out = torch.empty(K, dtype=torch.float32, device=y.device)
    if partial is None:
        partial = torch.empty(slots, 2, K, dtype=torch.float32, device=y.device)
    lib.check(lib.load().b200gnn_col_sum_f32(_f32(y, "y"), n, K, _f32(out, "out"), _f32(partial, "partial"), slots,
                                             lib.stream_ptr()), "col_sum_f32")
    return out


def bn_finalize(partial: torch.Tensor, n_rows: int, gamma, beta, eps: float = 1e-5, momentum: float = 0.1,
                running_mean=None, running_var=None, out: Optional[torch.Tensor] = None) -> torch.Tensor:
    slots, _, K = partial.shape
    if out is None:
        out = torch.empty(4, K, dtype=torch.float32, device=partial.device)
    lib.check(lib.load().b200gnn_bn_finalize_f32(
        _f32(partial, "partial"), slots, K, n_rows, _f32(gamma, "gamma"), _f32(beta, "beta"), eps, momentum,
        _f32(running_mean, "running_mean"), _f32(running_var, "running_var"),
        out[0].data_ptr(), out[1].data_ptr(), out[2].data_ptr(), out[3].data_ptr(), lib.stream_ptr()), "bn_finalize_f32")
    return out


def affine_relu_dropout(y: torch.Tensor, scale=None, shift=None, relu: bool = True, p: float = 0.0, seed: int = 0,
                        offset: int = 0, out: Optional[torch.Tensor] = None, step_dev: Optional[torch.Tensor] = None,
                        step_mul: int = 0, row_offset: int = 0) -> torch.Tensor:
    n, K = y.shape
    if out is None:
        out = torch.empty_like(y)
    lib.check(lib.load().b200gnn_affine_relu_dropout_f32(
        _f32(y, "y"), _f32(out, "out"), n, K, _f32(scale, "scale"), _f32(shift, "shift"), int(relu), p, seed, offset,
        lib.dptr(step_dev, torch.int32, "step_dev"), step_mul, row_offset, lib.stream_ptr()), "affine_relu_dropout_f32")
    return out


def affine_relu_dropout_mapped(y: torch.Tensor, scale=None, shift=None, relu: bool = True, p: float = 0.0, seed: int = 0,
                               offset: int = 0, out: Optional[torch.Tensor] = None, step_dev: Optional[torch.Tensor] = None,
                               step_mul: int = 0, rowmap: Optional[torch.Tensor] = None, row_offset: int = 0,
                               k_global: Optional[int] = None, col_offset: int = 0) -> torch.Tensor:
    n, K = y.shape
    if out is None:
        out = torch.empty_like(y)
    lib.check(lib.load().b200gnn_affine_relu_dropout_mapped_f32(
        _f32(y, "y"), _f32(out, "out"), n, K, _f32(scale, "scale"), _f32(shift, "shift"), int(relu), p, seed, offset,
        lib.dptr(step_dev, torch.int32, "step_dev"), step_mul, lib.dptr(rowmap, torch.int32, "rowmap"), row_offset,
        K if k_global is None else k_global, col_offset, lib.stream_ptr()), "affine_relu_dropout_mapped_f32")
    return out


def affine_relu_dropout_scatter(y: torch.Tensor, scale, shift, relu: bool, p: float, seed: int, offset: int, out: torch.Tensor,
                                step_dev, step_mul: int, rowmap, k_global: int, col_offset: int, dst_ptrs, row_off,
                                ld_dst: int) -> torch.Tensor:
    n, K = y.shape
    lib.check(lib.load().b200gnn_affine_relu_dropout_scatter_f32(
        _f32(y, "y"), _f32(out, "out"), n, K, _f32(scale, "scale"), _f32(shift, "shift"), int(relu), p, seed, offset,
        lib.dptr(step_dev, torch.int32, "step_dev"), step_mul, lib.dptr(rowmap, torch.int32, "rowmap"), 0, k_global, col_offset,
        _host_ptr_array(dst_ptrs), _host_i32_array(row_off), len(dst_ptrs), int(ld_dst), lib.stream_ptr()),
        "affine_relu_dropout_scatter_f32")
    return out


def dropout_mask(n_rows: int, K: int, p: float, seed: int, offset: int, device="cuda") -> torch.Tensor:
    mask = torch.empty(n_rows, K, dtype=torch.uint8, device=device)
    lib.check(lib.load().b200gnn_dropout_mask_u8(mask.data_ptr(), n_rows, K, p, seed, offset, lib.stream_ptr()),
              "dropout_mask_u8")
    return mask


def dropout_bits(bits: torch.Tensor, p: float, seed: int, offset: int, step_dev: Optional[torch.Tensor] = None,
                 step_mul: int = 0, K: Optional[int] = None) -> torch.Tensor:
    n_layers, n, words = bits.shape
    K = 32 * words if K is None else K
    assert bits.dtype == torch.int32 and bits.is_contiguous() and words == (K + 31) // 32
    lib.check(lib.load().b200gnn_dropout_bits_u32(bits.data_ptr(), n_layers, n, K, p, seed, offset,
                                                  lib.dptr(step_dev, torch.int32, "step_dev"), step_mul, lib.stream_ptr()),
              "dropout_bits_u32")
    return bits


def _bits(bits: torch.Tensor, n: int, K: int) -> int:
    if bits.dtype != torch.int32 or not bits.is_cuda or not bits.is_contiguous() or tuple(bits.shape) != (n, (K + 31) // 32):
        raise lib.B200GnnError(f"keep bits: expected a contiguous CUDA int32 [{n}, {(K + 31) // 32}] tensor")
    return bits.data_ptr()


def affine_relu_bits(y: torch.Tensor, bits: torch.Tensor, scale: torch.Tensor, shift: torch.Tensor, p: float,
                     out: Optional[torch.Tensor] = None) -> torch.Tensor:
    n, K = y.shape
    if out is None:
        out = torch.empty_like(y)
    lib.check(lib.load().b200gnn_affine_relu_bits_f32(_f32(y, "y"), _bits(bits, n, K), _f32(scale, "scale"), _f32(shift, "shift"),
                                                      p, _f32(out, "out"), n, K, lib.stream_ptr()), "affine_relu_bits_f32")
    return out


def bn_act_bwd(d_out, x_out, y, mean, invstd, gamma, p: float, d_y=None, d_gamma=None, d_beta=None, d_bias=None,
               partial=None, coef=None, want_dbias: bool = True):
    n, K = y.shape
    dev = y.device
    slots = rows_slots(n)
    d_y = torch.empty_like(y) if d_y is None else d_y
    d_gamma = torch.empty(K, device=dev) if d_gamma is None else d_gamma
    d_beta = torch.empty(K, device=dev) if d_beta is None else d_beta
    if want_dbias and d_bias is None:
        d_bias = torch.empty(K, device=dev)
    partial = torch.empty(slots, 2, K, device=dev) if partial is None else partial
    coef = torch.empty(3, K, device=dev) if coef is None else coef
    lib.check(lib.load().b200gnn_bn_act_bwd_f32(
        _f32(d_out, "d_out"), _f32(x_out, "x_out"), _f32(y, "y"), _f32(mean, "mean"), _f32(invstd, "invstd"),
        _f32(gamma, "gamma"), n, K, p, _f32(d_y, "d_y"), _f32(d_gamma, "d_gamma"), _f32(d_beta, "d_beta"),
        _f32(d_bias, "d_bias") if want_dbias else None, _f32(partial, "partial"), slots, _f32(coef, "coef"),
        lib.stream_ptr()), "bn_act_bwd_f32")
    return d_y, d_gamma, d_beta, d_bias


def adam_step(params, grads, exp_avg, exp_avg_sq, step: torch.Tensor, lr: float, betas=(0.9, 0.999), eps: float = 1e-8):
    lib.check(lib.load().b200gnn_adam_step_f32(
        _f32(params, "params"), _f32(grads, "grads"), _f32(exp_avg, "exp_avg"), _f32(exp_avg_sq, "exp_avg_sq"),
        params.numel(), lr, betas[0], betas[1], eps, lib.dptr(step, torch.int32, "step"), lib.stream_ptr()),
        "adam_step_f32")


def kd_loss_fwd_bwd(logits, labels, train_idx, teacher_logits=None, alpha: float = 0.9, T: float = 4.0,
                    d_logits=None, loss_out=None, partial=None, n_norm: int = 0):
    N, C = logits.shape
    n_train = train_idx.numel() if train_idx is not None else N
    L = lib.load()
    if d_logits is None:
        d_logits = torch.zeros_like(logits)
    if loss_out is None:
        loss_out = torch.empty(3, dtype=torch.float32, device=logits.device)
    if partial is None:
        partial = torch.empty(2 * int(L.b200gnn_kd_partials(max(n_train, 1))), dtype=torch.float32, device=logits.device)
    lib.check(L.b200gnn_kd_loss_fwd_bwd_f32(
        _f32(logits, "logits"), logits.stride(0), lib.dptr(train_idx, torch.int64, "train_idx"), n_train,
        lib.dptr(labels, torch.int64, "labels"), _f32(teacher_logits, "teacher_logits"),
        teacher_logits.stride(0) if teacher_logits is not None else 0, C, alpha, T, n_norm, _f32(d_logits, "d_logits"),
        d_logits.stride(0), _f32(loss_out, "loss_out"), _f32(partial, "partial"), lib.stream_ptr()), "kd_loss_fwd_bwd_f32")
    return loss_out, d_logits


def split_tf32(w: torch.Tensor, transpose: bool = False, hi: Optional[torch.Tensor] = None,
               lo: Optional[torch.Tensor] = None) -> Tuple[torch.Tensor, torch.Tensor]:
    rows, cols = w.shape
    shape = (cols, rows) if transpose else (rows, cols)
    hi = torch.empty(shape, dtype=torch.float32, device=w.device) if hi is None else hi
    lo = torch.empty(shape, dtype=torch.float32, device=w.device) if lo is None else lo
    lib.check(lib.load().b200gnn_split_tf32_f32(_f32(w, "w"), rows, cols, int(transpose), _f32(hi, "hi"), _f32(lo, "lo"),
                                                lib.stream_ptr()), "split_tf32_f32")
    return hi, lo


def gemm_tf32x3(a: torch.Tensor, b_hi: torch.Tensor, b_lo: torch.Tensor, bias: Optional[torch.Tensor] = None,
                out: Optional[torch.Tensor] = None, accumulate: bool = False) -> torch.Tensor:
    M, K = a.shape
    N = b_hi.shape[0]
    assert b_hi.shape == b_lo.shape and b_hi.shape[1] == K
    if out is None:
        assert not accumulate
        out = torch.empty(M, N, dtype=torch.float32, device=a.device)
    L = lib.load()
    if accumulate:
        assert bias is None
        lib.check(L.b200gnn_gemm_tf32x3_acc_f32(_f32(a, "a"), a.stride(0), _f32(b_hi, "b_hi"), _f32(b_lo, "b_lo"),
                                                b_hi.stride(0), _f32(out, "out"), out.stride(0), M, N, K, lib.stream_ptr()),
                  "gemm_tf32x3_acc_f32")
        return out
    lib.check(L.b200gnn_gemm_tf32x3_f32(_f32(a, "a"), a.stride(0), _f32(b_hi, "b_hi"), _f32(b_lo, "b_lo"),
                                        b_hi.stride(0), _f32(out, "out"), out.stride(0), M, N, K,
                                        _f32(bias, "bias"), lib.stream_ptr()), "gemm_tf32x3_f32")
    return out


def gemm_stat_slots(m: int, n: int) -> int:
    return int(lib.load().b200gnn_gemm_stat_slots(m, n))


def gemm_stats_supported(n: int) -> bool:
    return n % 32 == 0 and 48 < n <= 256


def gemm_tf32x3_stats(a: torch.Tensor, b_hi: torch.Tensor, b_lo: torch.Tensor, bias: Optional[torch.Tensor], out: torch.Tensor,
                      partial: torch.Tensor, accumulate: bool = False) -> torch.Tensor:
    M, K = a.shape
    N = b_hi.shape[0]
    lib.check(lib.load().b200gnn_gemm_tf32x3_stats_f32(_f32(a, "a"), a.stride(0), _f32(b_hi, "b_hi"), _f32(b_lo, "b_lo"),
                                                       b_hi.stride(0), _f32(out, "out"), out.stride(0), M, N, K, _f32(bias, "bias"),
                                                       int(accumulate), _f32(partial, "partial"), partial.shape[0], lib.stream_ptr()),
              "gemm_tf32x3_stats_f32")
    return out


def gemm_tf32x3_bnbwd(a: torch.Tensor, b_hi: torch.Tensor, b_lo: torch.Tensor, out: torch.Tensor, x_out: torch.Tensor,
                      y: torch.Tensor, mean: torch.Tensor, invstd: torch.Tensor, p: float, partial: torch.Tensor,
                      accumulate: bool = False) -> torch.Tensor:
    M, K = a.shape
    N = b_hi.shape[0]
    assert out.shape == x_out.shape == y.shape and out.stride(0) == x_out.stride(0) == y.stride(0)
    lib.check(lib.load().b200gnn_gemm_tf32x3_bnbwd_f32(_f32(a, "a"), a.stride(0), _f32(b_hi, "b_hi"), _f32(b_lo, "b_lo"),
                                                       b_hi.stride(0), _f32(out, "out"), out.stride(0), M, N, K, int(accumulate),
                                                       _f32(x_out, "x_out"), _f32(y, "y"), _f32(mean, "mean"),
                                                       _f32(invstd, "invstd"), float(p), _f32(partial, "partial"),
                                                       partial.shape[0], lib.stream_ptr()), "gemm_tf32x3_bnbwd_f32")
    return out


def gemm_tf32x3_bnbwd_bits(a: torch.Tensor, b_hi: torch.Tensor, b_lo: torch.Tensor, out: torch.Tensor, bits: torch.Tensor,
                           y: torch.Tensor, mean: torch.Tensor, invstd: torch.Tensor, scale: torch.Tensor, shift: torch.Tensor,
                           p: float, partial: torch.Tensor, accumulate: bool = False) -> torch.Tensor:
    M, K = a.shape
    N = b_hi.shape[0]
    assert out.shape == y.shape and out.stride(0) == y.stride(0)
    lib.check(lib.load().b200gnn_gemm_tf32x3_bnbwd_bits_f32(_f32(a, "a"), a.stride(0), _f32(b_hi, "b_hi"), _f32(b_lo, "b_lo"),
                                                            b_hi.stride(0), _f32(out, "out"), out.stride(0), M, N, K, int(accumulate),
                                                            _bits(bits, M, N), _f32(y, "y"), _f32(mean, "mean"), _f32(invstd, "invstd"),
                                                            _f32(scale, "scale"), _f32(shift, "shift"), float(p),
                                                            _f32(partial, "partial"), partial.shape[0], lib.stream_ptr()),
              "gemm_tf32x3_bnbwd_bits_f32")
    return out


def gemm_tf32x3_act(y: torch.Tensor, scale: torch.Tensor, shift: torch.Tensor, bits: torch.Tensor, p: float, b_hi: torch.Tensor,
                    b_lo: torch.Tensor, bias: Optional[torch.Tensor] = None, out: Optional[torch.Tensor] = None) -> torch.Tensor:
    M, K = y.shape
    N = b_hi.shape[0]
    assert b_hi.shape == b_lo.shape and b_hi.shape[1] == K
    if out is None:
        out = torch.empty(M, N, dtype=torch.float32, device=y.device)
    lib.check(lib.load().b200gnn_gemm_tf32x3_act_f32(_f32(y, "y"), y.stride(0), _f32(b_hi, "b_hi"), _f32(b_lo, "b_lo"),
                                                     b_hi.stride(0), _f32(out, "out"), out.stride(0), M, N, K, _f32(bias, "bias"),
                                                     _f32(scale, "scale"), _f32(shift, "shift"), _bits(bits, M, K), float(p),
                                                     lib.stream_ptr()), "gemm_tf32x3_act_f32")
    return out


def gemm_tf32x3_scatter(a: torch.Tensor, b_hi: torch.Tensor, b_lo: torch.Tensor, dst_ptrs, row_off: int,
                        bias: Optional[torch.Tensor] = None) -> None:
    import ctypes as C
    M, K = a.shape
    N = b_hi.shape[0]
    world = len(dst_ptrs)
    arr = (C.c_void_p * world)(*[C.c_void_p(int(p)) for p in dst_ptrs])
    lib.check(lib.load().b200gnn_gemm_tf32x3_scatter_f32(_f32(a, "a"), a.stride(0), _f32(b_hi, "b_hi"), _f32(b_lo, "b_lo"),
                                                         b_hi.stride(0), arr, world, int(row_off), M, N, K, _f32(bias, "bias"),
                                                         lib.stream_ptr()), "gemm_tf32x3_scatter_f32")


def gemm_tf32x3_bcast(a: torch.Tensor, b_hi: torch.Tensor, b_lo: torch.Tensor, dst_ptrs, row_off: int, ldc: int,
                      bias: Optional[torch.Tensor] = None) -> None:
    M, K = a.shape
    N = b_hi.shape[0]
    lib.check(lib.load().b200gnn_gemm_tf32x3_bcast_f32(_f32(a, "a"), a.stride(0), _f32(b_hi, "b_hi"), _f32(b_lo, "b_lo"),
                                                       b_hi.stride(0), _host_ptr_array(dst_ptrs), len(dst_ptrs), int(row_off), int(ldc),
                                                       M, N, K, _f32(bias, "bias"), lib.stream_ptr()), "gemm_tf32x3_bcast_f32")


def wgrad_supported(k_in: int, n_out: int) -> bool:
    return k_in in (128, 256) and n_out % 4 == 0 and 0 < n_out <= 256


def wgrad_workspace_floats(k_in: int, n_out: int) -> int:
    return int(lib.load().b200gnn_wgrad_workspace_floats(k_in, n_out))


def gemm_wgrad_tf32x3(x: torch.Tensor, g: torch.Tensor, out: Optional[torch.Tensor] = None,
                      workspace: Optional[torch.Tensor] = None, wide: bool = False) -> torch.Tensor:
    nn_, k_in = x.shape
    n_out = g.shape[1]
    assert g.shape[0] == nn_
    if not wide and not wgrad_supported(k_in, n_out):
        raise lib.B200GnnError(f"gemm_wgrad_tf32x3: Kin={k_in}, Nout={n_out} is outside the 128/256-row tilings "
                               "(pass wide=True for the padded ones)")
    L = lib.load()
    if out is None:
        out = torch.empty(k_in, n_out, dtype=torch.float32, device=x.device)
    if workspace is None:
        n_ws = int(L.b200gnn_wgrad_workspace_floats(k_in, n_out))
        if n_ws < 0:
            lib.check(n_ws, "wgrad_workspace_floats")
        workspace = torch.empty(n_ws, dtype=torch.float32, device=x.device)
    lib.check(L.b200gnn_gemm_wgrad_tf32x3_f32(_f32(x, "x"), x.stride(0), _f32(g, "g"), g.stride(0), _f32(out, "out"), nn_,
                                              k_in, n_out, _f32(workspace, "workspace"), lib.stream_ptr()),
              "gemm_wgrad_tf32x3_f32")
    return out


def gemm_wgrad_tf32x3_act(y: torch.Tensor, scale: torch.Tensor, shift: torch.Tensor, bits: torch.Tensor, p: float,
                          g: torch.Tensor, out: Optional[torch.Tensor] = None,
                          workspace: Optional[torch.Tensor] = None) -> torch.Tensor:
    nn_, k_in = y.shape
    n_out = g.shape[1]
    assert g.shape[0] == nn_
    if not wgrad_supported(k_in, n_out):
        raise lib.B200GnnError(f"gemm_wgrad_tf32x3_act: Kin={k_in}, Nout={n_out} is outside the 128/256-row tilings")
    L = lib.load()
    if out is None:
        out = torch.empty(k_in, n_out, dtype=torch.float32, device=y.device)
    if workspace is None:
        workspace = torch.empty(int(L.b200gnn_wgrad_workspace_floats(k_in, n_out)), dtype=torch.float32, device=y.device)
    lib.check(L.b200gnn_gemm_wgrad_tf32x3_act_f32(_f32(y, "y"), y.stride(0), _f32(g, "g"), g.stride(0), _f32(out, "out"), nn_,
                                                  k_in, n_out, _f32(scale, "scale"), _f32(shift, "shift"), _bits(bits, nn_, k_in),
                                                  float(p), _f32(workspace, "workspace"), lib.stream_ptr()),
              "gemm_wgrad_tf32x3_act_f32")
    return out


def partial_reduce(partial: torch.Tensor, out: Optional[torch.Tensor] = None) -> torch.Tensor:
    slots = partial.shape[0]
    k2 = partial.numel() // slots
    if out is None:
        out = torch.empty(partial.shape[1:], dtype=torch.float32, device=partial.device)
    lib.check(lib.load().b200gnn_partial_reduce_f32(_f32(partial, "partial"), slots, k2, _f32(out, "out"), lib.stream_ptr()),
              "partial_reduce_f32")
    return out


def bn_act_bwd_reduce(d_out, x_out, y, mean, invstd, p: float, partial: torch.Tensor) -> torch.Tensor:
    n, K = y.shape
    lib.check(lib.load().b200gnn_bn_act_bwd_reduce_f32(_f32(d_out, "d_out"), _f32(x_out, "x_out"), _f32(y, "y"),
                                                       _f32(mean, "mean"), _f32(invstd, "invstd"), n, K, p,
                                                       _f32(partial, "partial"), partial.shape[0], lib.stream_ptr()),
              "bn_act_bwd_reduce_f32")
    return partial


def bn_act_bwd_apply(d_out, x_out, y, mean, invstd, gamma, sums, n_norm: int, p: float, d_y, d_gamma, d_beta, d_bias,
                     partial, coef):
    n, K = y.shape
    sum_slots = sums.numel() // (2 * K)
    lib.check(lib.load().b200gnn_bn_act_bwd_apply_f32(
        _f32(d_out, "d_out"), _f32(x_out, "x_out"), _f32(y, "y"), _f32(mean, "mean"), _f32(invstd, "invstd"),
        _f32(gamma, "gamma"), _f32(sums, "sums"), sum_slots, n_norm, n, K, p, _f32(d_y, "d_y"), _f32(d_gamma, "d_gamma"),
        _f32(d_beta, "d_beta"), _f32(d_bias, "d_bias"), _f32(partial, "partial"), partial.shape[0], _f32(coef, "coef"),
        lib.stream_ptr()), "bn_act_bwd_apply_f32")


def relu_dropout_bwd(d_out: torch.Tensor, x_out: torch.Tensor, p: float, out: Optional[torch.Tensor] = None) -> torch.Tensor:
    n, K = x_out.shape
    assert d_out.shape == x_out.shape and d_out.is_contiguous() and x_out.is_contiguous()
    out = torch.empty_like(x_out) if out is None else out
    lib.check(lib.load().b200gnn_relu_dropout_bwd_f32(_f32(d_out, "d_out"), _f32(x_out, "x_out"), _f32(out, "out"), n, K, float(p),
                                                      lib.stream_ptr()), "relu_dropout_bwd_f32")
    return out


def _table_arrays(tables: dict, n_tables: int):
    import ctypes as C
    ptrs = (C.c_void_p * n_tables)()
    rows = (C.c_int64 * n_tables)()
    for k, t in tables.items():
        ptrs[k], rows[k] = t.data_ptr(), t.shape[0]
    return ptrs, rows


def typed_gather(tables: dict, n_tables: int, node_type: torch.Tensor, local_idx: torch.Tensor, out: torch.Tensor) -> torch.Tensor:
    ptrs, rows = _table_arrays(tables, n_tables)
    err = torch.zeros(1, dtype=torch.int32, device=out.device)
    lib.check(lib.load().b200gnn_typed_gather_f32(ptrs, rows, n_tables, lib.dptr(node_type, torch.int64, "node_type"),
                                                  lib.dptr(local_idx, torch.int64, "local_idx"), out.shape[0], out.shape[1],
                                                  _f32(out, "out"), out.stride(0), err.data_ptr(), lib.stream_ptr()),
              "typed_gather_f32")
    return out


def typed_scatter(d_out: torch.Tensor, node_type: torch.Tensor, local_idx: torch.Tensor, order: torch.Tensor, grads: dict,
                  n_tables: int) -> None:
    ptrs, rows = _table_arrays(grads, n_tables)
    lib.check(lib.load().b200gnn_typed_scatter_f32(_f32(d_out, "d_out"), d_out.stride(0), lib.dptr(node_type, torch.int64, "node_type"),
                                                   lib.dptr(local_idx, torch.int64, "local_idx"), lib.dptr(order, torch.int64, "order"),
                                                   d_out.shape[0], d_out.shape[1], ptrs, rows, n_tables, lib.stream_ptr()),
              "typed_scatter_f32")


def embedding_adam(d_out: torch.Tensor, node_type: torch.Tensor, local_idx: torch.Tensor, order: torch.Tensor, table_type: int,
                   table: torch.Tensor, exp_avg: torch.Tensor, exp_avg_sq: torch.Tensor, head: torch.Tensor, step: torch.Tensor,
                   lr: float, betas=(0.9, 0.999), eps: float = 1e-8) -> None:
    rows, F_ = table.shape
    assert exp_avg.shape == table.shape == exp_avg_sq.shape and head.numel() >= rows and d_out.shape[1] == F_
    lib.check(lib.load().b200gnn_embedding_adam_f32(
        _f32(d_out, "d_out"), d_out.stride(0), lib.dptr(node_type, torch.int64, "node_type"),
        lib.dptr(local_idx, torch.int64, "local_idx"), lib.dptr(order, torch.int64, "order"), d_out.shape[0], int(table_type),
        _f32(table, "table"), _f32(exp_avg, "exp_avg"), _f32(exp_avg_sq, "exp_avg_sq"), rows, F_,
        lib.dptr(head, torch.int32, "head"), lr, betas[0], betas[1], eps, lib.dptr(step, torch.int32, "step"), lib.stream_ptr()),
        "embedding_adam_f32")


def _rows(t: torch.Tensor, name: str):
    if not isinstance(t, torch.Tensor) or not t.is_cuda or t.dtype != torch.float32 or t.dim() != 2 or t.stride(1) != 1:
        raise lib.B200GnnError(f"{name}: expected a CUDA float32 matrix with contiguous rows")
    return t.data_ptr(), t.stride(0)


def _bits_rows(bits: torch.Tensor, n: int, K: int):
    if bits.dtype != torch.int32 or not bits.is_cuda or bits.dim() != 2 or bits.stride(1) != 1 or bits.shape[0] != n \
            or bits.shape[1] < (K + 31) // 32:
        raise lib.B200GnnError(f"keep bits: expected CUDA int32 [{n}, >= {(K + 31) // 32}] with contiguous rows")
    return bits.data_ptr(), bits.stride(0)


def prelu_bits(z: torch.Tensor, bits: torch.Tensor, slope: torch.Tensor, p: float, out: Optional[torch.Tensor] = None) -> torch.Tensor:
    n, K = z.shape
    if out is None:
        out = torch.empty(n, K, dtype=torch.float32, device=z.device)
    zp, ldz = _rows(z, "z")
    op, ldo = _rows(out, "out")
    bp, ldb = _bits_rows(bits, n, K)
    lib.check(lib.load().b200gnn_prelu_bits_f32(zp, ldz, bp, ldb, _f32(slope, "slope"), float(p), op, ldo, n, K, lib.stream_ptr()),
              "prelu_bits_f32")
    return out


def gemm_tf32x3_prelu(z: torch.Tensor, slope: torch.Tensor, bits: torch.Tensor, p: float, b_hi: torch.Tensor, b_lo: torch.Tensor,
                      bias: Optional[torch.Tensor] = None, out: Optional[torch.Tensor] = None) -> torch.Tensor:
    M, K = z.shape
    N = b_hi.shape[0]
    assert b_hi.shape == b_lo.shape and b_hi.shape[1] == K
    if out is None:
        out = torch.empty(M, N, dtype=torch.float32, device=z.device)
    zp, lda = _rows(z, "z")
    op, ldc = _rows(out, "out")
    if bits.shape[1] != (K + 31) // 32:
        raise lib.B200GnnError("gemm_tf32x3_prelu: keep bits must be [M, ceil(K/32)]")
    lib.check(lib.load().b200gnn_gemm_tf32x3_prelu_f32(zp, lda, _f32(b_hi, "b_hi"), _f32(b_lo, "b_lo"), b_hi.stride(0), op, ldc, M, N, K,
                                                       _f32(bias, "bias"), _f32(slope, "slope"), _bits(bits, M, K), float(p),
                                                       lib.stream_ptr()), "gemm_tf32x3_prelu_f32")
    return out


def gemm_tf32x3_prelu_bwd(a: torch.Tensor, b_hi: torch.Tensor, b_lo: torch.Tensor, out: torch.Tensor, z: torch.Tensor,
                          bits: torch.Tensor, slope: torch.Tensor, p: float, slope_grad: torch.Tensor, partial: torch.Tensor,
                          accumulate: bool = False, slope_accumulate: bool = False) -> torch.Tensor:
    M, K = a.shape
    N = b_hi.shape[0]
    assert out.shape == z.shape == (M, N) and out.stride(0) == z.stride(0)
    if partial.dtype != torch.float64 or not partial.is_cuda or partial.numel() < gemm_stat_slots(M, N):
        raise lib.B200GnnError("gemm_tf32x3_prelu_bwd: partial must be CUDA float64 [>= gemm_stat_slots(M, N)]")
    ap, lda = _rows(a, "a")
    op, ldc = _rows(out, "out")
    lib.check(lib.load().b200gnn_gemm_tf32x3_prelu_bwd_f32(ap, lda, _f32(b_hi, "b_hi"), _f32(b_lo, "b_lo"), b_hi.stride(0), op, ldc,
                                                           M, N, K, int(accumulate), _rows(z, "z")[0], _bits(bits, M, N),
                                                           _f32(slope, "slope"), float(p), slope_grad.data_ptr(),
                                                           int(slope_accumulate), partial.data_ptr(), partial.numel(),
                                                           lib.stream_ptr()), "gemm_tf32x3_prelu_bwd_f32")
    return out


WGRAD_PRELU_BLOCK = 512


def gemm_wgrad_tf32x3_prelu(z: torch.Tensor, slope: torch.Tensor, bits: torch.Tensor, p: float, g: torch.Tensor,
                            out: Optional[torch.Tensor] = None, workspace: Optional[torch.Tensor] = None) -> torch.Tensor:
    nn_, k_in = z.shape
    n_out = g.shape[1]
    assert g.shape[0] == nn_
    if k_in % 4 or n_out % 4:
        raise lib.B200GnnError(f"gemm_wgrad_tf32x3_prelu: Kin={k_in}, Nout={n_out} must be multiples of 4")
    L = lib.load()
    if out is None:
        out = torch.empty(k_in, n_out, dtype=torch.float32, device=z.device)
    blk = k_in if k_in <= 2048 else WGRAD_PRELU_BLOCK
    if workspace is None:
        workspace = torch.empty(wgrad_workspace_floats(blk, n_out), dtype=torch.float32, device=z.device)
    bp, ldb = _bits_rows(bits, nn_, k_in)
    gp, ldg = _rows(g, "g")
    assert out.is_contiguous()
    for c0 in range(0, k_in, blk):
        kb = min(blk, k_in - c0)
        zb, ldz = _rows(z[:, c0:c0 + kb], "z")
        lib.check(L.b200gnn_gemm_wgrad_tf32x3_prelu_f32(zb, ldz, gp, ldg, out[c0:c0 + kb].data_ptr(), nn_, kb, n_out,
                                                        _f32(slope, "slope"), bp + 4 * (c0 // 32), ldb, float(p),
                                                        _f32(workspace, "workspace"), lib.stream_ptr()),
                  "gemm_wgrad_tf32x3_prelu_f32")
    return out


def gemm_wgrad_tf32x3_rows(x: torch.Tensor, g: torch.Tensor, out: torch.Tensor, workspace: torch.Tensor) -> torch.Tensor:
    nn_, k_in = x.shape
    xp, ldx = _rows(x, "x")
    gp, ldg = _rows(g, "g")
    lib.check(lib.load().b200gnn_gemm_wgrad_tf32x3_f32(xp, ldx, gp, ldg, _f32(out, "out"), nn_, k_in, g.shape[1],
                                                       _f32(workspace, "workspace"), lib.stream_ptr()), "gemm_wgrad_tf32x3_f32")
    return out


def gemm_tf32x3_rows(a: torch.Tensor, b_hi: torch.Tensor, b_lo: torch.Tensor, out: torch.Tensor,
                     bias: Optional[torch.Tensor] = None) -> torch.Tensor:
    M, K = a.shape
    N = b_hi.shape[0]
    ap, lda = _rows(a, "a")
    op, ldc = _rows(out, "out")
    lib.check(lib.load().b200gnn_gemm_tf32x3_f32(ap, lda, _f32(b_hi, "b_hi"), _f32(b_lo, "b_lo"), b_hi.stride(0), op, ldc, M, N, K,
                                                 _f32(bias, "bias"), lib.stream_ptr()), "gemm_tf32x3_f32")
    return out


def col_sum_ld(y: torch.Tensor, out: torch.Tensor, partial: Optional[torch.Tensor] = None) -> torch.Tensor:
    n, K = y.shape
    L = lib.load()
    slots = int(L.b200gnn_col_sum_ld_slots(n))
    if partial is None:
        partial = torch.empty(slots * K, dtype=torch.float32, device=y.device)
    yp, ldy = _rows(y, "y")
    lib.check(L.b200gnn_col_sum_ld_f32(yp, ldy, n, K, _f32(out, "out"), partial.data_ptr(), partial.numel() // K, lib.stream_ptr()),
              "col_sum_ld_f32")
    return out


def sign_gather(feats, idx: torch.Tensor, p: float, seed: int, offset: int, out: torch.Tensor,
                step_dev: Optional[torch.Tensor] = None, step_mul: int = 0, labels: Optional[torch.Tensor] = None,
                labels_out: Optional[torch.Tensor] = None, teacher: Optional[torch.Tensor] = None,
                teacher_out: Optional[torch.Tensor] = None) -> torch.Tensor:
    H = len(feats)
    B = idx.numel()
    n, F_ = feats[0].shape
    for f in feats:
        if f.shape != (n, F_):
            raise lib.B200GnnError("sign_gather: every hop feature matrix must have the same shape")
        _f32(f, "feats")
    assert out.shape == (H, B, F_)
    C = teacher.shape[1] if teacher is not None else 0
    lib.check(lib.load().b200gnn_sign_gather_f32(
        _host_ptr_array([f.data_ptr() for f in feats]), H, n, F_, lib.dptr(idx, torch.int64, "idx"), B, float(p), int(seed),
        int(offset), lib.dptr(step_dev, torch.int32, "step_dev"), int(step_mul), _f32(out, "out"),
        lib.dptr(labels, torch.int64, "labels"), lib.dptr(labels_out, torch.int64, "labels_out"),
        _f32(teacher, "teacher"), teacher.stride(0) if teacher is not None else 0, C, _f32(teacher_out, "teacher_out"),
        lib.stream_ptr()), "sign_gather_f32")
    return out
```

### include/b200gnn.h

```cpp
#ifndef B200GNN_H_
#define B200GNN_H_

#include <stdint.h>

#ifdef __cplusplus
extern "C" {
#endif

#define B200GNN_OK 0
#define B200GNN_ERR_BAD_ARG (-1)
#define B200GNN_ERR_UNSUPPORTED (-2)
#define B200GNN_ERR_CUDA (-3)

#define B200GNN_REDUCE_SUM 0
#define B200GNN_REDUCE_MEAN 1

#define B200GNN_ABI_VERSION 2

int b200gnn_abi_version(void);
const char* b200gnn_error_string(int code);
const char* b200gnn_last_cuda_error(void);
int64_t b200gnn_launch_count(void);
void b200gnn_reset_launch_count(void);

int64_t b200gnn_csr_chunk_count(int64_t n_rows, int64_t nnz, int32_t chunk_nnz,
                                int32_t row_cost);
int b200gnn_csr_chunk_plan(const int32_t* rowptr, int64_t n_rows, int64_t nnz,
                           int32_t chunk_nnz, int32_t row_cost,
                           int32_t* chunk_rowptr, void* stream);

int b200gnn_csr_hub_count(const int32_t* rowptr, int64_t n_rows,
                          int32_t hub_threshold, int32_t seg_len,
                          int32_t* counts_out, void* stream);
int b200gnn_csr_hub_fill(const int32_t* rowptr, int64_t n_rows,
                         int32_t hub_threshold, int32_t seg_len,
                         int32_t* hub_rows, int32_t* hub_segptr,
                         int64_t n_hub, void* stream);

int64_t b200gnn_spmm_stat_slots(int64_t n_chunks, int64_t n_hub);
void b200gnn_spmm_set_variant(int variant);
int b200gnn_spmm_csr_f32(const int32_t* rowptr, const int32_t* col,
                         const float* val, const float* X, int64_t ldx,
                         float* Y, int64_t ldy, int64_t n_rows, int64_t n_src,
                         int64_t K, int reduce, const float* bias,
                         float* stat_partial, const int32_t* chunk_rowptr,
                         int64_t n_chunks, int32_t hub_threshold,
                         int32_t seg_len, const int32_t* hub_rows,
                         const int32_t* hub_segptr, int64_t n_hub,
                         int64_t n_seg, float* hub_workspace, void* stream);
int b200gnn_spmm_csr_scatter_f32(const int32_t* rowptr, const int32_t* col, const float* val, const float* X,
                                 int64_t ldx, float* const* Y_ptrs, const int32_t* row_off, int32_t world,
                                 int64_t ldy_dst, int64_t col_dst, int64_t n_rows, int64_t n_src, int64_t K,
                                 int reduce, const float* bias, const int32_t* chunk_rowptr, int64_t n_chunks,
                                 int32_t hub_threshold, int32_t seg_len, const int32_t* hub_rows,
                                 const int32_t* hub_segptr, int64_t n_hub, int64_t n_seg,
                                 float* hub_workspace, void* stream);

int64_t b200gnn_rows_slots(int64_t n_rows);
int b200gnn_col_stats_f32(const float* Y, int64_t n_rows, int64_t K,
                          float* partial, int64_t slots, void* stream);
int b200gnn_col_sum_f32(const float* Y, int64_t n_rows, int64_t K, float* out,
                        float* partial, int64_t slots, void* stream);
int b200gnn_bn_finalize_f32(const float* partial, int64_t slots, int64_t K,
                            int64_t n_rows, const float* gamma,
                            const float* beta, float eps, float momentum,
                            float* running_mean, float* running_var,
                            float* mean_out, float* invstd_out,
                            float* scale_out, float* shift_out, void* stream);
int b200gnn_affine_relu_dropout_f32(const float* Y, float* out, int64_t n_rows,
                                    int64_t K, const float* scale,
                                    const float* shift, int relu, float p,
                                    uint64_t seed, uint64_t offset,
                                    const int32_t* step_dev, uint64_t step_mul,
                                    uint64_t row_offset, void* stream);
int b200gnn_affine_relu_dropout_mapped_f32(const float* Y, float* out, int64_t n_rows, int64_t K,
                                           const float* scale, const float* shift, int relu, float p,
                                           uint64_t seed, uint64_t offset, const int32_t* step_dev,
                                           uint64_t step_mul, const int32_t* rowmap, uint64_t row_offset,
                                           int64_t K_global, int64_t col_offset, void* stream);
int b200gnn_affine_relu_dropout_scatter_f32(const float* Y, float* out, int64_t n_rows, int64_t K,
                                            const float* scale, const float* shift, int relu, float p,
                                            uint64_t seed, uint64_t offset, const int32_t* step_dev,
                                            uint64_t step_mul, const int32_t* rowmap, uint64_t row_offset,
                                            int64_t K_global, int64_t col_offset, float* const* dst_ptrs,
                                            const int32_t* row_off, int32_t world, int64_t ld_dst, void* stream);
int b200gnn_dropout_mask_u8(uint8_t* mask, int64_t n_rows, int64_t K, float p,
                            uint64_t seed, uint64_t offset, void* stream);
int b200gnn_dropout_bits_u32(uint32_t* bits, int64_t n_layers, int64_t n_rows, int64_t K, float p, uint64_t seed,
                             uint64_t offset, const int32_t* step_dev, uint64_t step_mul, void* stream);
int b200gnn_affine_relu_bits_f32(const float* Y, const uint32_t* bits, const float* scale, const float* shift,
                                 float p, float* out, int64_t n_rows, int64_t K, void* stream);
int b200gnn_relu_dropout_bwd_f32(const float* dOut, const float* Xout, float* dY,
                                 int64_t n_rows, int64_t K, float p, void* stream);
int b200gnn_bn_act_bwd_f32(const float* dOut, const float* Xout, const float* Y,
                           const float* mean, const float* invstd,
                           const float* gamma, int64_t n_rows, int64_t K,
                           float p, float* dY, float* dgamma, float* dbeta,
                           float* dbias, float* partial, int64_t slots,
                           float* coef, void* stream);
int b200gnn_bn_act_bwd_reduce_f32(const float* dOut, const float* Xout,
                                  const float* Y, const float* mean,
                                  const float* invstd, int64_t n_rows,
                                  int64_t K, float p, float* partial,
                                  int64_t slots, void* stream);
int b200gnn_bn_act_bwd_apply_f32(const float* dOut, const float* Xout,
                                 const float* Y, const float* mean,
                                 const float* invstd, const float* gamma,
                                 const float* sums, int64_t sum_slots,
                                 int64_t n_norm, int64_t n_rows, int64_t K,
                                 float p, float* dY, float* dgamma,
                                 float* dbeta, float* dbias, float* partial,
                                 int64_t slots, float* coef, void* stream);
int b200gnn_partial_reduce_f32(const float* partial, int64_t slots, int64_t K2,
                               float* out, void* stream);
int b200gnn_adam_step_f32(float* params, const float* grads, float* exp_avg,
                          float* exp_avg_sq, int64_t n, float lr, float beta1,
                          float beta2, float eps, int32_t* step, void* stream);

int64_t b200gnn_kd_partials(int64_t n_train);
int b200gnn_kd_loss_fwd_bwd_f32(const float* logits, int64_t ld,
                                const int64_t* train_idx, int64_t n_train,
                                const int64_t* labels,
                                const float* teacher_logits, int64_t ldt,
                                int64_t C, float alpha, float T,
                                int64_t n_norm, float* dlogits, int64_t ldd,
                                float* loss_out, float* partial, void* stream);

int b200gnn_split_tf32_f32(const float* W, int64_t rows, int64_t cols,
                           int transpose, float* hi, float* lo, void* stream);
int b200gnn_gemm_tf32x3_f32(const float* A, int64_t lda, const float* B_hi,
                            const float* B_lo, int64_t ldb, float* C,
                            int64_t ldc, int64_t M, int64_t N, int64_t K,
                            const float* bias, void* stream);
int b200gnn_gemm_tf32x3_acc_f32(const float* A, int64_t lda, const float* B_hi, const float* B_lo,
                                int64_t ldb, float* C, int64_t ldc, int64_t M, int64_t N, int64_t K,
                                void* stream);
int64_t b200gnn_gemm_stat_slots(int64_t M, int64_t N);
void b200gnn_gemm_set_bnbwd_variant(int v);
int b200gnn_gemm_tf32x3_stats_f32(const float* A, int64_t lda, const float* B_hi, const float* B_lo, int64_t ldb,
                                  float* C, int64_t ldc, int64_t M, int64_t N, int64_t K, const float* bias,
                                  int accumulate, float* partial, int64_t slots, void* stream);
int b200gnn_gemm_tf32x3_bnbwd_f32(const float* A, int64_t lda, const float* B_hi, const float* B_lo, int64_t ldb,
                                  float* C, int64_t ldc, int64_t M, int64_t N, int64_t K, int accumulate,
                                  const float* Xout, const float* Y, const float* mean, const float* invstd, float p_drop,
                                  float* partial, int64_t slots, void* stream);
int b200gnn_gemm_tf32x3_bnbwd_bits_f32(const float* A, int64_t lda, const float* B_hi, const float* B_lo, int64_t ldb,
                                       float* C, int64_t ldc, int64_t M, int64_t N, int64_t K, int accumulate,
                                       const uint32_t* bits, const float* Y, const float* mean, const float* invstd,
                                       const float* scale, const float* shift, float p_drop, float* partial,
                                       int64_t slots, void* stream);
int b200gnn_gemm_tf32x3_act_f32(const float* Y, int64_t lda, const float* B_hi, const float* B_lo, int64_t ldb,
                                float* C, int64_t ldc, int64_t M, int64_t N, int64_t K, const float* bias,
                                const float* scale, const float* shift, const uint32_t* bits, float p_drop,
                                void* stream);
int b200gnn_gemm_tf32x3_scatter_f32(const float* A, int64_t lda, const float* B_hi, const float* B_lo,
                                    int64_t ldb, float* const* C_ptrs, int32_t world, int64_t row_off,
                                    int64_t M, int64_t N, int64_t K, const float* bias, void* stream);
int b200gnn_gemm_tf32x3_bcast_f32(const float* A, int64_t lda, const float* B_hi, const float* B_lo,
                                  int64_t ldb, float* const* C_ptrs, int32_t world, int64_t row_off, int64_t ldc,
                                  int64_t M, int64_t N, int64_t K, const float* bias, void* stream);

int64_t b200gnn_wgrad_workspace_floats(int64_t Kin, int64_t Nout);
int b200gnn_gemm_wgrad_tf32x3_f32(const float* X, int64_t ldx, const float* G,
                                  int64_t ldg, float* dW, int64_t Nn,
                                  int64_t Kin, int64_t Nout, float* workspace,
                                  void* stream);
int b200gnn_gemm_wgrad_tf32x3_act_f32(const float* Y, int64_t ldx, const float* G, int64_t ldg, float* dW,
                                      int64_t Nn, int64_t Kin, int64_t Nout, const float* scale, const float* shift,
                                      const uint32_t* bits, float p_drop, float* workspace, void* stream);

int b200gnn_gemm_tf32x3_prelu_f32(const float* Z, int64_t lda, const float* B_hi, const float* B_lo, int64_t ldb,
                                  float* C, int64_t ldc, int64_t M, int64_t N, int64_t K, const float* bias,
                                  const float* slope, const uint32_t* bits, float p_drop, void* stream);
int b200gnn_gemm_tf32x3_prelu_bwd_f32(const float* A, int64_t lda, const float* B_hi, const float* B_lo, int64_t ldb,
                                      float* C, int64_t ldc, int64_t M, int64_t N, int64_t K, int accumulate,
                                      const float* Z, const uint32_t* bits, const float* slope, float p_drop,
                                      float* slope_grad, int slope_accumulate, double* partial, int64_t slots,
                                      void* stream);
int b200gnn_gemm_wgrad_tf32x3_prelu_f32(const float* Z, int64_t ldz, const float* G, int64_t ldg, float* dW,
                                        int64_t Nn, int64_t Kin, int64_t Nout, const float* slope,
                                        const uint32_t* bits, int64_t ldbits, float p_drop, float* workspace,
                                        void* stream);
int b200gnn_prelu_bits_f32(const float* Z, int64_t ldz, const uint32_t* bits, int64_t ldbits, const float* slope, float p,
                           float* out, int64_t ldo, int64_t n_rows, int64_t K, void* stream);
int b200gnn_sign_gather_f32(const float* const* feats, int32_t n_hops, int64_t n_nodes, int64_t F, const int64_t* idx,
                            int64_t B, float p, uint64_t seed, uint64_t offset, const int32_t* step_dev,
                            uint64_t step_mul, float* out, const int64_t* labels, int64_t* labels_out,
                            const float* teacher, int64_t ldt, int64_t C, float* teacher_out, void* stream);
int64_t b200gnn_col_sum_ld_slots(int64_t n_rows);
int b200gnn_col_sum_ld_f32(const float* Y, int64_t ldy, int64_t n_rows, int64_t K, float* out, float* partial,
                           int64_t slots, void* stream);

int b200gnn_row_normalize_fwd_f32(const float* x, int64_t n, int64_t F, float eps,
                                  float scale, float* out, float* norm_out,
                                  void* stream);
int b200gnn_row_normalize_bwd_f32(const float* out, const float* norm,
                                  const float* d_out, int64_t n, int64_t F,
                                  float eps, float scale, float* d_x,
                                  int accumulate, void* stream);
int64_t b200gnn_reduce_slots(int64_t n);
int b200gnn_mse_fwd_bwd_f32(const float* a, const float* b, int64_t n,
                            float grad_weight, float* d_a, float* loss_out,
                            float* partial, void* stream);
int b200gnn_bce_logits_fwd_bwd_f32(const float* z, const float* target,
                                   int target_is_logits, int64_t n,
                                   float grad_weight, float* d_z, float* loss_out,
                                   float* partial, void* stream);
int b200gnn_row_sqnorm_f32(const float* x, int64_t n, int64_t F, float* out, void* stream);
int b200gnn_row_sqnorm_bwd_f32(const float* x, const float* d_out, int64_t n,
                               int64_t F, float* d_x, void* stream);
int b200gnn_nce_rows_f32(float* Z, int64_t S, float* loss_out, float* partial, void* stream);
int b200gnn_nce_rows_chunk_f32(float* Z, int64_t ldz, int64_t n_rows, int64_t S, int64_t row_offset,
                               float* partial, void* stream);
int b200gnn_nce_finish_f32(const float* partial, int64_t S, float* loss_out, void* stream);
int b200gnn_transpose_f32(const float* in, int64_t rows, int64_t cols, float* out, void* stream);
int b200gnn_gsp_pair_f32(float* Gs, const float* Gt, const float* ns, const float* nt,
                         int64_t S, int kernel, float* rowcoef, float* loss_out,
                         float* partial, void* stream);
int b200gnn_row_axpy_f32(const float* x, const float* coef, int64_t n, int64_t F,
                         float alpha, float* y, void* stream);

int b200gnn_edge_sim_f32(const float* feat, int64_t F, const int32_t* src,
                         const int32_t* dst, int64_t E, int kernel, float* sim,
                         void* stream);
int64_t b200gnn_lsp_partials(int64_t n_seg);
int b200gnn_lsp_segment_f32(const float* sim_s, const float* sim_t,
                            const int32_t* rowptr, int64_t n_seg, int64_t E,
                            int criterion, float* g, float* loss_out,
                            float* partial, void* stream);
int b200gnn_edge_sim_bwd_f32(const float* feat, int64_t F, const int32_t* src,
                             const int32_t* dst, int64_t E, int kernel,
                             const float* sim, const float* g, float* dfeat,
                             void* stream);
int b200gnn_lsp_bwd_values_f32(const float* feat, int64_t F, const int32_t* src, const int32_t* dst,
                               int64_t E, int kernel, const float* sim, const float* g,
                               const int32_t* pos_dst, const int32_t* pos_src,
                               const int32_t* comb_rowptr, const int32_t* diag_pos, int64_t n_nodes,
                               float* val, float* selfc, void* stream);

int b200gnn_gat_edge_softmax_f32(const int32_t* rowptr, const int32_t* col,
                                 const float* el, const float* er, int64_t n_rows,
                                 int64_t H, float negative_slope, float softmax_eps,
                                 float* a, const uint8_t* edge_keep, void* stream);
int b200gnn_gat_aggregate_f32(const int32_t* rowptr, const int32_t* col,
                              const int32_t* eidx, const float* a, const float* ft,
                              int64_t ldf, float* out, int64_t ldo, int64_t n_rows,
                              int64_t H, int64_t D, const int32_t* chunk_rowptr,
                              int64_t n_chunks, int32_t hub_threshold, int32_t seg_len,
                              const int32_t* hub_rows, const int32_t* hub_segptr,
                              int64_t n_hub, int64_t n_seg, float* hub_workspace,
                              void* stream);
int b200gnn_gat_bwd_rows_f32(const int32_t* rowptr, const int32_t* col, const float* a,
                             const float* ft, int64_t ldf, const float* dout,
                             int64_t ldd, const float* el, const float* er,
                             int64_t n_rows, int64_t H, int64_t D,
                             float negative_slope, float* dpre, float* der,
                             const int32_t* chunk_rowptr, int64_t n_chunks,
                             int32_t hub_threshold, int32_t seg_len,
                             const int32_t* hub_rows, const int32_t* hub_segptr,
                             int64_t n_hub, int64_t n_seg, float* hub_workspace,
                             const float* attn_scale, void* stream);
int b200gnn_segment_sum_heads_f32(const int32_t* rowptr, const int32_t* eidx,
                                  const float* vals, int64_t n_rows, int64_t H,
                                  float* out, void* stream);

typedef struct b200gnn_copy2d {
  float* dst;
  const float* src;
  int64_t ld_dst;
  int64_t ld_src;
  int64_t rows;
} b200gnn_copy2d;
int b200gnn_arena_alloc(int64_t bytes, void** out);
int b200gnn_arena_free(void* ptr);
int b200gnn_ipc_get_handle(const void* dev_ptr, void* handle64);
int b200gnn_ipc_open_handle(const void* handle64, void** out);
int b200gnn_ipc_close_handle(void* ptr);
int b200gnn_peer_copy2d_f32(const b200gnn_copy2d* copies, int32_t n, int64_t width, void* stream);
int b200gnn_peer_barrier(uint64_t* const* peer_flags, int32_t rank, int32_t world,
                         uint64_t* epoch, int32_t* error, void* stream);
int b200gnn_peer_exchange_f32(const b200gnn_copy2d* copies, int32_t n, int64_t width,
                              uint64_t* const* peer_flags, int32_t rank, int32_t world, uint64_t* epoch,
                              int32_t* error, uint32_t* ticket, void* stream);

int b200gnn_typed_gather_f32(const float* const* tables, const int64_t* table_rows, int32_t n_tables,
                             const int64_t* node_type, const int64_t* local_idx, int64_t n, int64_t F,
                             float* out, int64_t ldo, int32_t* error_flag, void* stream);
int b200gnn_embedding_adam_f32(const float* d_out, int64_t ldd, const int64_t* node_type,
                               const int64_t* local_idx, const int64_t* order, int64_t n,
                               int64_t table_type, float* table, float* exp_avg, float* exp_avg_sq,
                               int64_t rows, int64_t F, int32_t* head, float lr, float beta1,
                               float beta2, float eps, const int32_t* step, void* stream);
int b200gnn_typed_scatter_f32(const float* d_out, int64_t ldd, const int64_t* node_type,
                              const int64_t* local_idx, const int64_t* order, int64_t n, int64_t F,
                              float* const* d_tables, const int64_t* table_rows, int32_t n_tables,
                              void* stream);

int64_t b200gnn_graph_sort_workspace_bytes(int64_t n);
int b200gnn_graph_argsort_i64(const int64_t* major, const int64_t* minor, int64_t n, int64_t major_size,
                              int64_t minor_size, int32_t* perm_out, void* workspace, void* stream);
int b200gnn_graph_coalesce_i64(const int64_t* row, const int64_t* col, int64_t n, int64_t n_rows,
                               int64_t n_cols, int64_t* out_row, int64_t* out_col, int32_t* src_out,
                               int64_t* rowptr_out, int64_t* nnz_out, void* workspace, void* stream);

int b200gnn_random_walk_i64(const int32_t* rowptr, const int32_t* col, int64_t n_nodes, const int64_t* start,
                            int64_t n_walks, int32_t walk_length, uint64_t seed, uint64_t offset, int64_t* out,
                            void* stream);
int b200gnn_saint_subgraph_count_i64(const int32_t* rowptr, const int32_t* col, const int64_t* nodes, int64_t n_sel,
                                     int32_t* node_map, int64_t* counts, void* stream);
int b200gnn_saint_subgraph_fill_i64(const int32_t* rowptr, const int32_t* col, const int64_t* eid, const int64_t* nodes,
                                    int64_t n_sel, const int32_t* node_map, const int64_t* out_ptr, int64_t* out_row,
                                    int64_t* out_col, int64_t* out_eid, void* stream);

#ifdef __cplusplus
}
#endif
#endif
```

Measured before the change: 3.462 billion.

## Fold layer-0 batchnorm backward into the weight-gradient GEMM prologue

For the first layer in agg-first mode, the BN backward dY computation is moved into the TF32x3 weight-gradient kernel. That kernel now TMA-loads Y alongside dz, computes dY in shared memory before splitting, and accumulates per-slot bias column sums as chains. The goal is to drop a separate elementwise pass that reads dz and Y and writes dY over the whole node×256 matrix. The cost is fewer pipeline stages (3 instead of 5) for the extra Y buffer, release of the stage buffer moved after the wgmma issue, and extra kernels to reduce the bias chains.

Result: slower. 3.323 billion (median of 6 runs) (-4.0%).

```diff
diff --git a/efficient-gnns_b200/csrc/common.cuh b/efficient-gnns_b200/csrc/common.cuh
--- a/efficient-gnns_b200/csrc/common.cuh
+++ b/efficient-gnns_b200/csrc/common.cuh
@@ -27,6 +27,10 @@
   const float vi = b2 * v + (1.f - b2) * g * g;
   m = mi; v = vi;
   p -= step_size * mi / (sqrtf(vi) * inv_sqrt_bc2 + eps);
+}
+
+__device__ __forceinline__ float bn_bwd_dy(float dz, float y, float mu, float is, float c1, float c2, float c3) {
+  return __fmul_rn(c1, __fmaf_rn(-c3, __fmul_rn(__fsub_rn(y, mu), is), __fsub_rn(dz, c2)));
 }
 
 template <typename V> struct VecTraits;
diff --git a/efficient-gnns_b200/csrc/dense_rows.cu b/efficient-gnns_b200/csrc/dense_rows.cu
--- a/efficient-gnns_b200/csrc/dense_rows.cu
+++ b/efficient-gnns_b200/csrc/dense_rows.cu
@@ -351,10 +351,10 @@
         g.z = x.z > 0.f ? g.z * inv_keep : 0.f; g.w = x.w > 0.f ? g.w * inv_keep : 0.f;
       }
       float4 d;
-      d.x = c1.x * (g.x - c2.x - (y.x - mu.x) * is.x * c3.x);
-      d.y = c1.y * (g.y - c2.y - (y.y - mu.y) * is.y * c3.y);
-      d.z = c1.z * (g.z - c2.z - (y.z - mu.z) * is.z * c3.z);
-      d.w = c1.w * (g.w - c2.w - (y.w - mu.w) * is.w * c3.w);
+      d.x = bn_bwd_dy(g.x, y.x, mu.x, is.x, c1.x, c2.x, c3.x);
+      d.y = bn_bwd_dy(g.y, y.y, mu.y, is.y, c1.y, c2.y, c3.y);
+      d.z = bn_bwd_dy(g.z, y.z, mu.z, is.z, c1.z, c2.z, c3.z);
+      d.w = bn_bwd_dy(g.w, y.w, mu.w, is.w, c1.w, c2.w, c3.w);
       st4(dY + o, d);
       s.x += d.x; s.y += d.y; s.z += d.z; s.w += d.w;
     }
@@ -601,6 +601,21 @@
   return B200GNN_OK;
 }
 
+extern "C" int b200gnn_bn_bwd_finalize_f32(const float* sums, int64_t sum_slots, int64_t n_norm, int64_t K, const float* gamma,
+                                           const float* invstd, float* dgamma, float* dbeta, float* coef, void* stream) {
+  if (!sums || !gamma || !invstd || !dgamma || !dbeta || !coef || sum_slots < 1 || n_norm < 1 || K < 1 || K > INT32_MAX)
+    return B200GNN_ERR_BAD_ARG;
+  bn_bwd_finalize_kernel<<<(int)((K + FIN_COLS - 1) / FIN_COLS), 256, 0, (cudaStream_t)stream>>>(
+      sums, (int)sum_slots, (int)K, n_norm, gamma, invstd, dgamma, dbeta, coef);
+  return check_launch();
+}
+
+extern "C" int b200gnn_colsum_finalize_f32(const float* partial, int64_t slots, int64_t K, float* out, void* stream) {
+  if (!partial || !out || slots < 1 || K < 1 || K > INT32_MAX) return B200GNN_ERR_BAD_ARG;
+  colsum_finalize_kernel<<<(int)((K + FIN_COLS - 1) / FIN_COLS), 256, 0, (cudaStream_t)stream>>>(partial, (int)slots, (int)K, out);
+  return check_launch();
+}
+
 extern "C" int b200gnn_bn_act_bwd_f32(const float* dOut, const float* Xout, const float* Y, const float* mean,
                                       const float* invstd, const float* gamma, int64_t n_rows, int64_t K, float p,
                                       float* dY, float* dgamma, float* dbeta, float* dbias, float* partial,
diff --git a/efficient-gnns_b200/csrc/gemm_wgrad_tf32x3.cu b/efficient-gnns_b200/csrc/gemm_wgrad_tf32x3.cu
--- a/efficient-gnns_b200/csrc/gemm_wgrad_tf32x3.cu
+++ b/efficient-gnns_b200/csrc/gemm_wgrad_tf32x3.cu
@@ -8,17 +8,20 @@
 constexpr int BKN = 32;
 constexpr int TM = 128, TN = 128;
 constexpr int THREADS = 384;
-constexpr int STAGES = 5;
 constexpr int X_BOX = 8;
-constexpr int RAW_BYTES = BKN * (TM + TN) * 4;
 constexpr int OP_BYTES = 128 * BKN * 4;
 constexpr int T_BYTES = 2 * OP_BYTES;
 constexpr int SS_BYTES = TM / 2 * 16;
-constexpr int SMEM_BYTES = STAGES * RAW_BYTES + 2 * T_BYTES + 256 + SS_BYTES + 1024;
+template <bool BNG>
+struct Lay {
+  static constexpr int STAGES = BNG ? 3 : 5;
+  static constexpr int RAW_BYTES = BKN * (TM + (BNG ? 2 : 1) * TN) * 4;
+  static constexpr int SMEM_BYTES = STAGES * RAW_BYTES + 2 * T_BYTES + 256 + SS_BYTES + 1024;
+  static_assert(SMEM_BYTES <= 232448, "shared memory");
+};
 constexpr int MAX_RANGES = 132;
 constexpr int64_t MAX_PARTIAL_FLOATS = (int64_t)MAX_RANGES * 256 * 256;
 constexpr int MAX_KIN = 2048, MAX_NOUT = 512;
-static_assert(SMEM_BYTES <= 232448, "shared memory");
 
 struct Params {
   float* partial;
@@ -31,11 +34,21 @@
   float inv_keep;
   const float* act_slope;
   int32_t act_ld;
+  const float* bn_mean;
+  const float* bn_invstd;
+  const float* bn_coef;
+  const float* bn_dz;
+  const float* bn_y;
+  int64_t bn_ld;
+  int32_t bn_per;
+  float* chains;
 };
 
-template <bool ACT, bool PRELU = false>
+template <bool ACT, bool PRELU = false, bool BNG = false>
 __global__ void __launch_bounds__(THREADS, 1)
-wgrad_tf32x3_kernel(const __grid_constant__ CUtensorMap tmX, const __grid_constant__ CUtensorMap tmG, const Params p) {
+wgrad_tf32x3_kernel(const __grid_constant__ CUtensorMap tmX, const __grid_constant__ CUtensorMap tmG,
+                    const __grid_constant__ CUtensorMap tmY, const Params p) {
+  constexpr int STAGES = Lay<BNG>::STAGES, RAW_BYTES = Lay<BNG>::RAW_BYTES;
   extern __shared__ uint8_t smem_raw[];
   uint8_t* smem = reinterpret_cast<uint8_t*>((reinterpret_cast<uintptr_t>(smem_raw) + 1023) & ~(uintptr_t)1023);
   uint8_t* tbuf = smem + STAGES * RAW_BYTES;
@@ -67,6 +80,7 @@
         for (int j = 0; j < TM / X_BOX; ++j)
           tma_load_2d(&tmX, &full[s], st + j * BKN * X_BOX * 4, mt * TM + j * X_BOX, kb * BKN);
         tma_load_2d(&tmG, &full[s], st + BKN * TM * 4, nt * TN, kb * BKN);
+        if (BNG) tma_load_2d(&tmY, &full[s], st + BKN * (TM + TN) * 4, nt * TN, kb * BKN);
         if (++s == STAGES) { s = 0; ph ^= 1; }
       }
     }
@@ -98,6 +112,29 @@
     if (kb0 < kb1) wnext = act_word(kb0);
     named_sync(1, 256);
   }
+  const int gcol = nt * TN + (ct & 127), half = ct >> 7;
+  float bmu = 0.f, bis = 0.f, bc1 = 0.f, bc2 = 0.f, bc3 = 0.f;
+  if (BNG && gcol < p.Nout) {
+    bmu = __ldg(p.bn_mean + gcol); bis = __ldg(p.bn_invstd + gcol);
+    bc1 = __ldg(p.bn_coef + gcol); bc2 = __ldg(p.bn_coef + p.Nout + gcol); bc3 = __ldg(p.bn_coef + 2 * p.Nout + gcol);
+  }
+  const int range_lo = kb0 * BKN, range_hi = min(kb1 * BKN, p.Nn);
+  int slot_lo = (range_lo + p.bn_per - 1) / p.bn_per * p.bn_per;
+  int slot_hi = min(slot_lo + p.bn_per, p.Nn);
+  float ch0 = 0.f, ch1 = 0.f;
+  auto chain_row = [&](int row, float v) {
+    const int g = (row - slot_lo) & 3;
+    if ((g >> 1) == half) { if (g & 1) ch1 += v; else ch0 += v; }
+    if (row + 1 == slot_hi) {
+      if (gcol < p.Nout) {
+        float* o = p.chains + ((size_t)(slot_lo / p.bn_per) * 4 + 2 * half) * p.Nout + gcol;
+        o[0] = ch0; o[p.Nout] = ch1;
+      }
+      ch0 = ch1 = 0.f;
+      slot_lo = slot_hi; slot_hi = min(slot_lo + p.bn_per, p.Nn);
+    }
+  };
+  const bool sums = BNG && mt == 0;
   float acc[64], sum[64];
 #pragma unroll
   for (int i = 0; i < 64; ++i) sum[i] = acc[i] = 0.f;
@@ -118,15 +155,26 @@
     }
     if (PRELU) asm volatile("" : "+r"(l4));
     const uint32_t sraw = smem_u32(smem + s * RAW_BYTES);
-    const float* rg = reinterpret_cast<const float*>(smem + s * RAW_BYTES + BKN * TM * 4);
+    float* rg = reinterpret_cast<float*>(smem + s * RAW_BYTES + BKN * TM * 4);
     uint8_t* T = tbuf + (i & 1) * T_BYTES;
 #pragma unroll
     for (int u = 0; u < 4; ++u) {
       const int idx = u * 256 + ct;
       const int r = idx & 127, c = idx >> 7;
-      const float* src = rg + (4 * c) * 128 + r;
-      const uint4 v = make_uint4(__float_as_uint(src[0]), __float_as_uint(src[128]), __float_as_uint(src[256]),
-                                 __float_as_uint(src[384]));
+      float* src = rg + (4 * c) * 128 + r;
+      uint4 v = make_uint4(__float_as_uint(src[0]), __float_as_uint(src[128]), __float_as_uint(src[256]),
+                           __float_as_uint(src[384]));
+      if (BNG) {
+        const float* ys = src + BKN * TN;
+        const int node = (kb0 + i) * BKN + 4 * c;
+        const bool col_ok = gcol < p.Nout;
+        const float d0 = col_ok && node < p.Nn ? bn_bwd_dy(src[0], ys[0], bmu, bis, bc1, bc2, bc3) : 0.f;
+        const float d1 = col_ok && node + 1 < p.Nn ? bn_bwd_dy(src[128], ys[128], bmu, bis, bc1, bc2, bc3) : 0.f;
+        const float d2 = col_ok && node + 2 < p.Nn ? bn_bwd_dy(src[256], ys[256], bmu, bis, bc1, bc2, bc3) : 0.f;
+        const float d3 = col_ok && node + 3 < p.Nn ? bn_bwd_dy(src[384], ys[384], bmu, bis, bc1, bc2, bc3) : 0.f;
+        src[0] = d0; src[128] = d1; src[256] = d2; src[384] = d3;
+        v = make_uint4(__float_as_uint(d0), __float_as_uint(d1), __float_as_uint(d2), __float_as_uint(d3));
+      }
       uint4 hv, lv;
       split4(v, hv, lv);
       *reinterpret_cast<uint4*>(T + swz128(r, c)) = hv;
@@ -150,8 +198,10 @@
         }
         split1(v, h[k][j], l[k][j]);
       }
-    asm volatile("fence.proxy.async.shared::cta;" ::: "memory");
-    mbar_arrive(&empty[s]);
+    if (!BNG) {
+      asm volatile("fence.proxy.async.shared::cta;" ::: "memory");
+      mbar_arrive(&empty[s]);
+    }
     if (i > 0) {
       wgmma_wait<0>();
       acc_fence(acc);
@@ -171,6 +221,17 @@
 #pragma unroll
     for (int k = 0; k < BKN / 8; ++k) wgmma_tf32_n128_rs(acc, h[k], make_desc_k128(sa + k * 32), 1);
     wgmma_commit();
+    if (BNG) {
+      const int node0 = (kb0 + i) * BKN;
+      if (sums)
+        for (int j = 0; j < BKN; ++j) {
+          const int row = node0 + j;
+          if (row >= p.Nn) break;
+          if (row >= slot_lo) chain_row(row, rg[j * 128 + (ct & 127)]);
+        }
+      asm volatile("fence.proxy.async.shared::cta;" ::: "memory");
+      mbar_arrive(&empty[s]);
+    }
     if (++s == STAGES) { s = 0; ph ^= 1; }
   };
   for (int i = 0; i < kb1 - kb0; i += 2) {
@@ -182,6 +243,23 @@
     acc_fence(acc);
 #pragma unroll
     for (int j = 0; j < 64; ++j) sum[j] += acc[j];
+  }
+  if (sums && slot_lo < range_hi) {
+    const int end = slot_hi;
+    for (int r0 = range_hi; r0 < end; r0 += 16) {
+      float v[16];
+#pragma unroll
+      for (int u = 0; u < 16; ++u) {
+        v[u] = 0.f;
+        if (r0 + u < end && gcol < p.Nout) {
+          const size_t o = (size_t)(r0 + u) * p.bn_ld + gcol;
+          v[u] = bn_bwd_dy(__ldg(p.bn_dz + o), __ldg(p.bn_y + o), bmu, bis, bc1, bc2, bc3);
+        }
+      }
+#pragma unroll
+      for (int u = 0; u < 16; ++u)
+        if (r0 + u < end) chain_row(r0 + u, v[u]);
+    }
   }
   float* out = p.partial + (size_t)range * p.Kpad * p.Npad;
   const int row0 = mt * TM + cw * 64 + (warp & 3) * 16 + (lane >> 2);
@@ -252,23 +330,25 @@
   return wgrad::range_cap(Kin, Nout) * wgrad::pad_k(Kin) * wgrad::pad_n(Nout);
 }
 
-template <bool ACT, bool PRELU = false>
+template <bool ACT, bool PRELU = false, bool BNG = false>
 static int wgrad_launch(const float* X, int64_t ldx, const float* G, int64_t ldg, float* dW, int64_t Nn, int64_t Kin, int64_t Nout,
-                        float* workspace, const wgrad::Params& act, void* stream) {
+                        float* workspace, const wgrad::Params& act, void* stream, const float* Ybn = nullptr) {
   if (!X || !G || !dW || !workspace || Nn <= 0 || Kin <= 0 || Nout <= 0 || ldx < Kin || ldg < Nout || Nn >= INT32_MAX)
     return B200GNN_ERR_BAD_ARG;
   if (Kin % 4 || Kin > wgrad::MAX_KIN || Nout % 4 || Nout > wgrad::MAX_NOUT || ldx % 4 || ldg % 4 || !aligned_to(X, 16) || !aligned_to(G, 16) ||
       !aligned_to(dW, 16) || !aligned_to(workspace, 16))
     return B200GNN_ERR_UNSUPPORTED;
-  CUtensorMap tX, tG;
+  CUtensorMap tX, tG, tY;
   if (!wgrad::make_map_rows(&tX, X, Nn, Kin, ldx, wgrad::X_BOX) || !wgrad::make_map_rows(&tG, G, Nn, Nout, ldg, wgrad::TN))
     return B200GNN_ERR_UNSUPPORTED;
+  tY = tG;
+  if (BNG && !wgrad::make_map_rows(&tY, Ybn, Nn, Nout, ldg, wgrad::TN)) return B200GNN_ERR_UNSUPPORTED;
   int dev = 0, sms = 132;
   cudaGetDevice(&dev);
   static bool attr_set[64] = {};
   if (dev >= 0 && dev < 64 && !attr_set[dev]) {
-    cudaError_t e = cudaFuncSetAttribute(wgrad::wgrad_tf32x3_kernel<ACT, PRELU>, cudaFuncAttributeMaxDynamicSharedMemorySize,
-                                         wgrad::SMEM_BYTES);
+    cudaError_t e = cudaFuncSetAttribute(wgrad::wgrad_tf32x3_kernel<ACT, PRELU, BNG>, cudaFuncAttributeMaxDynamicSharedMemorySize,
+                                         wgrad::Lay<BNG>::SMEM_BYTES);
     if (e != cudaSuccess) { set_cuda_error(e); return B200GNN_ERR_CUDA; }
     attr_set[dev] = true;
   }
@@ -288,7 +368,7 @@
   if (ranges < 1) ranges = 1;
   p.n_ranges = ranges;
   int rc;
-  wgrad::wgrad_tf32x3_kernel<ACT, PRELU><<<tiles * ranges, wgrad::THREADS, wgrad::SMEM_BYTES, st>>>(tX, tG, p);
+  wgrad::wgrad_tf32x3_kernel<ACT, PRELU, BNG><<<tiles * ranges, wgrad::THREADS, wgrad::Lay<BNG>::SMEM_BYTES, st>>>(tX, tG, tY, p);
   if ((rc = check_launch())) return rc;
   const int64_t n_vec = (int64_t)p.Kpad * p.Npad / 4;
   wgrad::wgrad_reduce_kernel<<<(int)((n_vec + wgrad::RED_VECS - 1) / wgrad::RED_VECS), wgrad::RED_VECS * wgrad::RED_GROUPS, 0, st>>>(
@@ -296,6 +376,43 @@
   return check_launch();
 }
 
+namespace b200gnn {
+namespace wgrad {
+__global__ void __launch_bounds__(256) bias_chains_kernel(const float* __restrict__ chains, int slots, int live, int Nout,
+                                                          float* __restrict__ partial) {
+  const int i = blockIdx.x * 256 + threadIdx.x;
+  if (i >= slots * Nout) return;
+  const int sl = i / Nout, c = i - sl * Nout;
+  float a = 0.f;
+  if (sl < live) {
+    const float* ch = chains + (size_t)sl * 4 * Nout + c;
+    a += ch[0]; a += ch[Nout]; a += ch[2 * Nout]; a += ch[3 * Nout];
+  }
+  partial[(size_t)sl * 2 * Nout + c] = a;
+  partial[(size_t)sl * 2 * Nout + Nout + c] = 0.f;
+}
+}
+}
+
+extern "C" int b200gnn_gemm_wgrad_tf32x3_bnbwd_f32(const float* X, int64_t ldx, const float* dz, const float* Y, int64_t ldg,
+                                                   float* dW, int64_t Nn, int64_t Kin, int64_t Nout, const float* mean,
+                                                   const float* invstd, const float* coef, float* dbias, float* bias_partial,
+                                                   int64_t partial_floats, float* workspace, void* stream) {
+  if (!dz || !Y || !mean || !invstd || !coef || !dbias || !bias_partial || Nn <= 0 || Nn >= INT32_MAX) return B200GNN_ERR_BAD_ARG;
+  const int64_t slots = b200gnn_rows_slots(Nn), per = (Nn + slots - 1) / slots;
+  if (partial_floats < slots * 6 * Nout) return B200GNN_ERR_BAD_ARG;
+  if (Nout != 256 || !aligned_to(Y, 16)) return B200GNN_ERR_UNSUPPORTED;
+  wgrad::Params bn{};
+  bn.bn_mean = mean; bn.bn_invstd = invstd; bn.bn_coef = coef; bn.bn_dz = dz; bn.bn_y = Y; bn.bn_ld = ldg;
+  bn.bn_per = (int32_t)per; bn.chains = bias_partial + slots * 2 * Nout;
+  int rc = wgrad_launch<false, false, true>(X, ldx, dz, ldg, dW, Nn, Kin, Nout, workspace, bn, stream, Y);
+  if (rc) return rc;
+  const int live = (int)((Nn + per - 1) / per);
+  wgrad::bias_chains_kernel<<<(int)((slots * Nout + 255) / 256), 256, 0, (cudaStream_t)stream>>>(
+      bn.chains, (int)slots, live, (int)Nout, bias_partial);
+  if ((rc = check_launch())) return rc;
+  return b200gnn_colsum_finalize_f32(bias_partial, slots, Nout, dbias, stream);
+}
 extern "C" int b200gnn_gemm_wgrad_tf32x3_f32(const float* X, int64_t ldx, const float* G, int64_t ldg, float* dW,
                                              int64_t Nn, int64_t Kin, int64_t Nout, float* workspace, void* stream) {
   return wgrad_launch<false>(X, ldx, G, ldg, dW, Nn, Kin, Nout, workspace, wgrad::Params{}, stream);
diff --git a/efficient-gnns_b200/engine.py b/efficient-gnns_b200/engine.py
--- a/efficient-gnns_b200/engine.py
+++ b/efficient-gnns_b200/engine.py
@@ -142,6 +142,8 @@
         self._static: Dict[str, torch.Tensor] = {}
         for k in set(dims[1:]):
             self._part(k); self._coef(k)
+        self._wgrad_bias_part = (torch.empty(ops.wgrad_bnbwd_partial_floats(N, dims[1]), device=dev)
+                                 if self.agg_first and dims[1] == 256 else None)
 
     def reset_parameters(self, seed: int = 0):
         g = torch.Generator().manual_seed(seed)
@@ -261,13 +263,17 @@
 
     def backward(self, x: torch.Tensor, d_out_feat: Optional[torch.Tensor] = None):
         fused = self._fwd_fused
+        fold_dy0 = False
         for l in range(self.L - 1, -1, -1):
             act = self._act(l - 1) if fused and l > 0 else None
             inp = x if l == 0 else (None if act else self._A[l - 1])
             if l == self.L - 1:
                 ops.col_sum(self.dY[l], out=self.gb[l], partial=self._part(self.dims[l + 1]))
             if l == 0 and self.agg_first:
-                self._wgrad_async(0, self.AX, self.dY[0])
+                if fold_dy0:
+                    self._wgrad_async(0, self.AX, self.dA[0], bn=True)
+                else:
+                    self._wgrad_async(0, self.AX, self.dY[0])
                 continue
             ops.spmm_csr(self.Gt, self.dY[l], "sum", out=self.dH[l])
             d_prev = self.dA[l - 1] if l > 0 else None
@@ -290,7 +296,11 @@
             if l > 0:
                 k = self.dims[l]
                 part = self._part(k)
-                if gp is not None:
+                if gp is not None and l == 1 and self._wgrad_bias_part is not None and self.wgrad_ws is not None \
+                        and ops.wgrad_supported(self.dims[0], self.dims[1]):
+                    ops.bn_bwd_finalize(gp, self.N, self.gamma[0], self.bn[0][1], self.ggamma[0], self.gbeta[0], self._coef(k))
+                    fold_dy0 = True
+                elif gp is not None:
                     ops.bn_act_bwd_apply(d_prev, None, self.Y[l - 1], self.bn[l - 1][0], self.bn[l - 1][1], self.gamma[l - 1],
                                          gp, self.N, self.p, self.dY[l - 1], self.ggamma[l - 1], self.gbeta[l - 1],
                                          self.gb[l - 1], part, self._coef(k))
@@ -300,13 +310,13 @@
                                    d_beta=self.gbeta[l - 1], d_bias=self.gb[l - 1], partial=part, coef=self._coef(k))
         self._wgrad_join()
 
-    def _wgrad_async(self, l: int, inp: Optional[torch.Tensor], d_out: torch.Tensor, act=None):
+    def _wgrad_async(self, l: int, inp: Optional[torch.Tensor], d_out: torch.Tensor, act=None, bn: bool = False):
         if self._side is None:
-            return self._linear_wgrad(l, inp, d_out, act)
+            return self._linear_wgrad(l, inp, d_out, act, bn)
         self._ev_fork.record(torch.cuda.current_stream())
         self._side.wait_event(self._ev_fork)
         with torch.cuda.stream(self._side):
-            self._linear_wgrad(l, inp, d_out, act)
+            self._linear_wgrad(l, inp, d_out, act, bn)
 
     def _wgrad_join(self):
         if self._side is not None:
@@ -334,8 +344,12 @@
         else:
             torch.mm(d_out, self.W[l].t(), out=d_inp)
 
-    def _linear_wgrad(self, l: int, inp: Optional[torch.Tensor], d_out: torch.Tensor, act=None):
-        if act is not None:
+    def _linear_wgrad(self, l: int, inp: Optional[torch.Tensor], d_out: torch.Tensor, act=None, bn: bool = False):
+        if bn:
+            ops.gemm_wgrad_tf32x3_bnbwd(inp, d_out, self.Y[l], self.bn[l][0], self.bn[l][1], self._coef(self.dims[l + 1]),
+                                        out=self.gW[l], d_bias=self.gb[l], bias_partial=self._wgrad_bias_part,
+                                        workspace=self.wgrad_ws)
+        elif act is not None:
             ops.gemm_wgrad_tf32x3_act(*act, self.p, d_out, out=self.gW[l], workspace=self.wgrad_ws)
         elif self.tc_gemm and ops.wgrad_supported(self.dims[l], self.dims[l + 1]):
             ops.gemm_wgrad_tf32x3(inp, d_out, out=self.gW[l], workspace=self.wgrad_ws)
diff --git a/efficient-gnns_b200/lib.py b/efficient-gnns_b200/lib.py
--- a/efficient-gnns_b200/lib.py
+++ b/efficient-gnns_b200/lib.py
@@ -59,6 +59,8 @@
     "b200gnn_bn_act_bwd_apply_f32": (_int, [_f32p, _f32p, _f32p, _f32p, _f32p, _f32p, _f32p, _i64, _i64, _i64, _i64, _f32,
                                             _f32p, _f32p, _f32p, _f32p, _f32p, _i64, _f32p, _ptr]),
     "b200gnn_partial_reduce_f32": (_int, [_f32p, _i64, _i64, _f32p, _ptr]),
+    "b200gnn_bn_bwd_finalize_f32": (_int, [_f32p, _i64, _i64, _i64, _f32p, _f32p, _f32p, _f32p, _f32p, _ptr]),
+    "b200gnn_colsum_finalize_f32": (_int, [_f32p, _i64, _i64, _f32p, _ptr]),
     "b200gnn_adam_step_f32": (_int, [_f32p, _f32p, _f32p, _f32p, _i64, _f32, _f32, _f32, _f32, _i32p, _ptr]),
     "b200gnn_kd_partials": (_i64, [_i64]),
     "b200gnn_kd_loss_fwd_bwd_f32": (_int, [_f32p, _i64, _ptr, _i64, _ptr, _f32p, _i64, _i64, _f32, _f32, _i64, _f32p,
@@ -85,6 +87,8 @@
     "b200gnn_gemm_wgrad_tf32x3_f32": (_int, [_f32p, _i64, _f32p, _i64, _f32p, _i64, _i64, _i64, _f32p, _ptr]),
     "b200gnn_gemm_wgrad_tf32x3_act_f32": (_int, [_f32p, _i64, _f32p, _i64, _f32p, _i64, _i64, _i64, _f32p, _f32p, _ptr, _f32,
                                                  _f32p, _ptr]),
+    "b200gnn_gemm_wgrad_tf32x3_bnbwd_f32": (_int, [_f32p, _i64, _f32p, _f32p, _i64, _f32p, _i64, _i64, _i64, _f32p, _f32p,
+                                                   _f32p, _f32p, _f32p, _i64, _f32p, _ptr]),
     "b200gnn_gemm_tf32x3_prelu_f32": (_int, [_f32p, _i64, _f32p, _f32p, _i64, _f32p, _i64, _i64, _i64, _i64, _f32p,
                                              _f32p, _ptr, _f32, _ptr]),
     "b200gnn_gemm_tf32x3_prelu_bwd_f32": (_int, [_f32p, _i64, _f32p, _f32p, _i64, _f32p, _i64, _i64, _i64, _i64, _int,
diff --git a/efficient-gnns_b200/ops.py b/efficient-gnns_b200/ops.py
--- a/efficient-gnns_b200/ops.py
+++ b/efficient-gnns_b200/ops.py
@@ -426,6 +426,29 @@
     return out
 
 
+def wgrad_bnbwd_partial_floats(n: int, n_out: int) -> int:
+    return rows_slots(n) * 6 * n_out
+
+
+def gemm_wgrad_tf32x3_bnbwd(x: torch.Tensor, dz: torch.Tensor, y: torch.Tensor, mean: torch.Tensor, invstd: torch.Tensor,
+                            coef: torch.Tensor, out: torch.Tensor, d_bias: torch.Tensor, bias_partial: torch.Tensor,
+                            workspace: Optional[torch.Tensor] = None) -> torch.Tensor:
+    nn_, k_in = x.shape
+    n_out = dz.shape[1]
+    assert dz.shape == y.shape and dz.shape[0] == nn_ and dz.stride(0) == y.stride(0)
+    if not wgrad_supported(k_in, n_out):
+        raise lib.B200GnnError(f"gemm_wgrad_tf32x3_bnbwd: Kin={k_in}, Nout={n_out} is outside the 128/256-row tilings")
+    L = lib.load()
+    if workspace is None:
+        workspace = torch.empty(int(L.b200gnn_wgrad_workspace_floats(k_in, n_out)), dtype=torch.float32, device=x.device)
+    lib.check(L.b200gnn_gemm_wgrad_tf32x3_bnbwd_f32(_f32(x, "x"), x.stride(0), _f32(dz, "dz"), _f32(y, "y"), dz.stride(0),
+                                                    _f32(out, "out"), nn_, k_in, n_out, _f32(mean, "mean"), _f32(invstd, "invstd"),
+                                                    _f32(coef, "coef"), _f32(d_bias, "d_bias"), _f32(bias_partial, "bias_partial"),
+                                                    bias_partial.numel(), _f32(workspace, "workspace"), lib.stream_ptr()),
+              "gemm_wgrad_tf32x3_bnbwd_f32")
+    return out
+
+
 def partial_reduce(partial: torch.Tensor, out: Optional[torch.Tensor] = None) -> torch.Tensor:
     slots = partial.shape[0]
     k2 = partial.numel() // slots
@@ -454,6 +477,15 @@
         _f32(gamma, "gamma"), _f32(sums, "sums"), sum_slots, n_norm, n, K, p, _f32(d_y, "d_y"), _f32(d_gamma, "d_gamma"),
         _f32(d_beta, "d_beta"), _f32(d_bias, "d_bias"), _f32(partial, "partial"), partial.shape[0], _f32(coef, "coef"),
         lib.stream_ptr()), "bn_act_bwd_apply_f32")
+
+
+def bn_bwd_finalize(sums: torch.Tensor, n_norm: int, gamma: torch.Tensor, invstd: torch.Tensor, d_gamma: torch.Tensor,
+                    d_beta: torch.Tensor, coef: torch.Tensor) -> torch.Tensor:
+    K = gamma.shape[0]
+    lib.check(lib.load().b200gnn_bn_bwd_finalize_f32(_f32(sums, "sums"), sums.numel() // (2 * K), n_norm, K, _f32(gamma, "gamma"),
+                                                     _f32(invstd, "invstd"), _f32(d_gamma, "d_gamma"), _f32(d_beta, "d_beta"),
+                                                     _f32(coef, "coef"), lib.stream_ptr()), "bn_bwd_finalize_f32")
+    return coef
 
 
 def relu_dropout_bwd(d_out: torch.Tensor, x_out: torch.Tensor, p: float, out: Optional[torch.Tensor] = None) -> torch.Tensor:
diff --git a/include/b200gnn.h b/include/b200gnn.h
--- a/include/b200gnn.h
+++ b/include/b200gnn.h
@@ -111,6 +111,9 @@
                                  float p, float* dY, float* dgamma,
                                  float* dbeta, float* dbias, float* partial,
                                  int64_t slots, float* coef, void* stream);
+int b200gnn_bn_bwd_finalize_f32(const float* sums, int64_t sum_slots, int64_t n_norm, int64_t K, const float* gamma,
+                                const float* invstd, float* dgamma, float* dbeta, float* coef, void* stream);
+int b200gnn_colsum_finalize_f32(const float* partial, int64_t slots, int64_t K, float* out, void* stream);
 int b200gnn_partial_reduce_f32(const float* partial, int64_t slots, int64_t K2,
                                float* out, void* stream);
 int b200gnn_adam_step_f32(float* params, const float* grads, float* exp_avg,
@@ -168,6 +171,10 @@
 int b200gnn_gemm_wgrad_tf32x3_act_f32(const float* Y, int64_t ldx, const float* G, int64_t ldg, float* dW,
                                       int64_t Nn, int64_t Kin, int64_t Nout, const float* scale, const float* shift,
                                       const uint32_t* bits, float p_drop, float* workspace, void* stream);
+int b200gnn_gemm_wgrad_tf32x3_bnbwd_f32(const float* X, int64_t ldx, const float* dz, const float* Y, int64_t ldg,
+                                        float* dW, int64_t Nn, int64_t Kin, int64_t Nout, const float* mean,
+                                        const float* invstd, const float* coef, float* dbias, float* bias_partial,
+                                        int64_t partial_floats, float* workspace, void* stream);
 
 int b200gnn_gemm_tf32x3_prelu_f32(const float* Z, int64_t lda, const float* B_hi, const float* B_lo, int64_t ldb,
                                   float* C, int64_t ldc, int64_t M, int64_t N, int64_t K, const float* bias,
```
